# lks1248/SPH-EXA

Hardware: AMD Instinct MI355X
Metric: particle-updates/sec (whole node), Sedov -n 400, 1/2/4/8 MI355X + HBM roofline % (higher is better)
Workload: dtype f32 hydro / f64 coordinates (sph::SphTypes)

## Files before the change

### include/sphexa_hip.h

```cpp
#ifndef SPHEXA_HIP_H
#define SPHEXA_HIP_H

#include <stddef.h>
#include <stdint.h>

#ifdef __cplusplus
extern "C" {
#endif

#define SX_OK 0
#define SX_ERR_TRAVERSAL 1
#define SX_ERR_NOT_CONVERGED 2
#define SX_ERR_HIP 3
#define SX_ERR_ARG 4
#define SX_ERR_NOMEM 5

typedef struct sx_box
{
    double  lim[6];
    int32_t bnd[3];
} sx_box;

typedef struct sx_params
{
// ... 10 lines not shown
    int32_t  avClean;
    float    theta;
    double   g;
    double   eps, etaAcc;
    int32_t  propagator;
} sx_params;

typedef struct sx_fields
{
    size_t    n;
    double *  x, *y, *z;
    float *   x_m1, *y_m1, *z_m1;
    float *   vx, *vy, *vz;
    float*    rho;
    double*   u;
    float *   p, *prho, *tdpdTrho, *h, *m, *c;
    float *   ax, *ay, *az;
    double*   du;
    float*    du_m1;
    float *   c11, *c12, *c13, *c22, *c23, *c33;
    float *   mue, *mui;
    double*   temp;
    float *   cv, *xm, *kx, *divv, *curlv, *alpha, *gradh;
    uint64_t* keys;
    uint32_t* nc;
    float *   dV11, *dV12, *dV13, *dV22, *dV23, *dV33;
    float*    markRamp;
    uint8_t*  rung;
} sx_fields;

typedef struct sx_tree
{
    int32_t         numLeafNodes;
    int32_t         numNodes;
    const uint64_t* prefixes;
    const int32_t*  childOffsets;
    const int32_t*  internalToLeaf;
    const int32_t*  levelRange;
    const uint64_t* leaves;
    const uint32_t* layout;
    const double*   centers;
    const double*   sizes;
    float           searchExtFactor;
} sx_tree;

typedef struct sx_groups
{
    uint32_t        firstBody, lastBody, numGroups;
    const uint32_t* groupStart;
    const uint32_t* groupEnd;
} sx_groups;

typedef struct sx_octree
{
    uint64_t* prefixes;
    int32_t*  childOffsets;
    int32_t*  parents;
    int32_t*  levelRange;
    int32_t*  internalToLeaf;
    int32_t*  leafToInternal;
} sx_octree;

typedef struct sx_nbstats
{
    uint64_t sumNeighbors;
    uint32_t maxNeighbors;
    uint32_t numFailed;
    uint64_t sumCandidates;
    uint64_t sumUnion;
    uint32_t build;
    uint32_t maxUnion;
} sx_nbstats;

typedef struct sx_ctx sx_ctx;

int         sx_create(sx_ctx** ctx, int device);
void        sx_destroy(sx_ctx* ctx);
int         sx_set_stream(sx_ctx* ctx, void* hipStream);
void*       sx_get_stream(sx_ctx* ctx);
const char* sx_last_error(sx_ctx* ctx);
int    sx_set_exact(sx_ctx* ctx, int exact);
double sx_kernel_constant(void);
int    sx_kernel_poly(const float* v, size_t n, float* w, float* dw);
int    sx_copy_tables(sx_ctx* ctx, float* wh_host, float* whd_host);
int    sx_synchronize(sx_ctx* ctx);

void* sx_device_alloc(sx_ctx* ctx, size_t bytes);
int   sx_device_free(sx_ctx* ctx, void* ptr);
int   sx_memcpy(sx_ctx* ctx, void* dst, const void* src, size_t bytes, int kind);
int   sx_memset(sx_ctx* ctx, void* dst, int value, size_t bytes);

int sx_sfc_keys(sx_ctx* ctx, const double* x, const double* y, const double* z, uint64_t* keys, size_t n,
                const sx_box* box);
int sx_sort_keys(sx_ctx* ctx, uint64_t* keys, uint32_t* order, size_t n);
int sx_gather(sx_ctx* ctx, const uint32_t* order, size_t n, const void* src, void* dst, int elemBytes);
int sx_compute_octree(sx_ctx* ctx, const uint64_t* sortedKeys, size_t n, uint32_t bucketSize, uint64_t* leaves,
                      uint32_t* counts, int32_t capacity, int32_t* numLeaves);
int sx_build_octree(sx_ctx* ctx, const uint64_t* leaves, int32_t numLeaves, const sx_octree* out);
int sx_node_centers(sx_ctx* ctx, const uint64_t* prefixes, int32_t numNodes, const sx_box* box, double* centers,
                    double* sizes);
int sx_leaf_layout(sx_ctx* ctx, const uint32_t* counts, int32_t numLeaves, uint32_t* layout);

int sx_compute_groups(sx_ctx* ctx, uint32_t first, uint32_t last, sx_groups* groups);
int sx_spatial_groups(sx_ctx* ctx, uint32_t first, uint32_t last, const double* x, const double* y, const double* z,
                      const sx_tree* tree, const sx_box* box, float tolFactor, uint32_t* groups, uint32_t cap,
                      sx_groups* out);
int sx_set_search_mode(sx_ctx* ctx, int mode);
int sx_find_neighbors(sx_ctx* ctx, const sx_fields* f, const sx_tree* tree, const sx_box* box,
                      const sx_params* p, uint32_t first, uint32_t last, int iterate_h, sx_nbstats* stats);
int sx_export_neighbors(sx_ctx* ctx, const uint32_t* nc, uint32_t first, uint32_t last, uint32_t ngmax,
                        uint32_t* neighbors);
int sx_import_neighbors(sx_ctx* ctx, uint32_t first, uint32_t last, uint32_t ngmax, const uint32_t* neighbors);

int sx_xmass(sx_ctx* ctx, const sx_groups* g, const sx_fields* f, const sx_params* p, const sx_box* box,
             const sx_tree* tree);
int sx_xmass_only(sx_ctx* ctx, const sx_groups* g, const sx_fields* f, const sx_params* p, const sx_box* box);
int sx_ve_def_gradh(sx_ctx* ctx, const sx_groups* g, const sx_fields* f, const sx_params* p, const sx_box* box);
int sx_eos(sx_ctx* ctx, uint32_t first, uint32_t last, float mui, double gamma, const double* temp, const float* m,
           const float* kx, const float* xm, const float* gradh, float* prho, float* c, float* rho, float* p);
int sx_iad_divv_curlv(sx_ctx* ctx, const sx_groups* g, const sx_fields* f, const sx_params* p, const sx_box* box);
int sx_av_switches(sx_ctx* ctx, const sx_groups* g, const sx_fields* f, const sx_params* p, const sx_box* box,
                   double minDt);
int sx_momentum_energy(sx_ctx* ctx, const sx_groups* g, float* groupDt, const sx_fields* f, const sx_params* p,
                       const sx_box* box, float* minDtCourant);
int sx_momentum_energy_avclean(sx_ctx* ctx, const sx_groups* g, float* groupDt, const sx_fields* f,
                               const sx_params* p, const sx_box* box, float* minDtCourant);
int sx_density(sx_ctx* ctx, const sx_groups* g, const sx_fields* f, const sx_params* p, const sx_box* box,
               const sx_tree* tree);
int sx_density_only(sx_ctx* ctx, const sx_groups* g, const sx_fields* f, const sx_params* p, const sx_box* box);
int sx_eos_std(sx_ctx* ctx, uint32_t first, uint32_t last, float mui, double gamma, const double* temp,
               const float* m, float* rho, float* p, float* c);
int sx_iad(sx_ctx* ctx, const sx_groups* g, const sx_fields* f, const sx_params* p, const sx_box* box);
int sx_momentum_energy_std(sx_ctx* ctx, const sx_groups* g, const sx_fields* f, const sx_params* p,
                           const sx_box* box, float* minDtCourant);

int sx_positions(sx_ctx* ctx, uint32_t first, uint32_t last, double dt, double dt_m1, const sx_fields* f,
                 double gamma, float muiConst, const sx_box* box);
int sx_update_h(sx_ctx* ctx, uint32_t first, uint32_t last, uint32_t ng0, const uint32_t* nc, float* h);
int sx_update_h_groups(sx_ctx* ctx, const sx_groups* g, uint32_t ng0, const uint32_t* nc, float* h);

int sx_mark_ramp(sx_ctx* ctx, const sx_groups* g, const sx_fields* f, const sx_params* p, const sx_box* box,
                 float* markRamp);

#define SX_MAX_RUNGS 4
int sx_positions_rungs(sx_ctx* ctx, const sx_groups* g, float dt, const float* dt_m1, const uint8_t* rung,
                       const sx_fields* f, double gamma, double constCv, const sx_box* box);
int sx_drift_positions(sx_ctx* ctx, const sx_groups* g, float dt, float dt_back, const float* dt_m1,
                       const uint8_t* rung, const sx_fields* f, double gamma, double constCv);
int sx_group_divv_timestep(sx_ctx* ctx, float Krho, const sx_groups* g, const float* divv, float* groupDt);
int sx_group_acc_timestep(sx_ctx* ctx, float etaAcc, const sx_groups* g, const float* ax, const float* ay,
                          const float* az, float* groupDt);
int sx_store_rung(sx_ctx* ctx, const sx_groups* g, uint8_t rung, uint8_t* rungs);
int sx_max_divv(sx_ctx* ctx, uint32_t first, uint32_t last, const float* divv, float* maxDivv);

int sx_conserved_quantities(sx_ctx* ctx, const sx_fields* f, uint32_t first, uint32_t last, float muiConst,
                            double gamma, double out[9]);

int sx_gravity_upsweep(sx_ctx* ctx, const sx_fields* f, const sx_tree* tree, float theta, double* centers,
                       float* multipoles);
int sx_gravity_traverse(sx_ctx* ctx, const sx_groups* g, const sx_fields* f, const sx_tree* tree, const sx_box* box,
                        const double* centers, const float* multipoles, float G, double* egrav);
int sx_gravity_traverse_pbc(sx_ctx* ctx, const sx_groups* g, const sx_fields* f, const sx_tree* tree,
                            const sx_box* box, const double* centers, const float* multipoles, float G, int numShells,
                            double* egrav);

typedef struct
// ... 116 lines not shown
```

### sph-exa_amd/csrc/sx_capi.cpp

```cpp
#include <hip/hip_runtime.h>

#include <algorithm>
#include <cmath>
#include <cstdio>
#include <cstring>
#include <string>
#include <vector>

#include "../../include/sphexa_hip.h"
#include "sx_comm.hpp"
#include "sx_gravity.hpp"
#include "sx_hydro.hpp"
#include "sx_kernel_poly.hpp"
#include "sx_observables.hpp"
#include "sx_tree.hpp"
#include "sx_timestep.hpp"
#include "sx_turb.hpp"

using namespace sx;

namespace
{

double wharmonic(double v)
{
    if (v == 0.0) return 1.0;
    const double Pv = M_PI_2 * v;
    return std::sin(Pv) / Pv;
}

double wharmonicDerivative(double v)
{
    if (v == 0.0) return 0.0;
    const double Pv    = M_PI_2 * v;
    const double sincv = std::sin(Pv) / Pv;
    return sincv * M_PI_2 * ((std::cos(Pv) / std::sin(Pv)) - 1.0 / Pv);
}

double sinc6(double x) { return std::pow(wharmonic(x), 6.0); }
double sinc6d(double x) { return 6.0 * std::pow(wharmonic(x), 6.0 - 1) * wharmonicDerivative(x); }
double kvol(double x) { return 4.0 * M_PI * x * x * sinc6(x); }

double simpsonK()
{
    const uint64_t n = 2000;
    double a = 0, b = 2.0, h = (b - a) / double(n);
    std::vector<double> odd(n / 2), even(n / 2 - 1);
    for (uint64_t i = 0; i < odd.size(); ++i)
        odd[i] = kvol(a + double(2 * (i + 1) - 1) * h);
    for (uint64_t i = 0; i < even.size(); ++i)
        even[i] = kvol(a + double(2 * (i + 1)) * h);
    std::sort(odd.begin(), odd.end());
    std::sort(even.begin(), even.end());
    double so = 0, se = 0;
    for (double v : odd)
        so += v;
    for (double v : even)
        se += v;
    return 1.0 / (h / 3.0 * (kvol(a) + kvol(b) + 4.0 * so + 2.0 * se));
}

void makeTables(std::vector<float>& wh, std::vector<float>& whd)
{
    wh.resize(kTableSize);
    whd.resize(kTableSize);
    const float dx = (float)((2.0 - 0.0) / (kTableSize - 1));
    for (size_t i = 0; i < (size_t)kTableSize; ++i)
    {
        float nv = (float)(0.0 + (float)i * dx);
        wh[i]    = (float)sinc6((double)nv);
        whd[i]   = (float)sinc6d((double)nv);
    }
}

DevBox toDev(const sx_box* b)
{
    DevBox d{};
    for (int k = 0; k < 6; ++k)
        d.lim[k] = b->lim[k];
    d.anyPbc = 0;
    for (int k = 0; k < 3; ++k)
    {
        d.l[k]   = b->lim[2 * k + 1] - b->lim[2 * k];
        d.il[k]  = 1.0 / (b->lim[2 * k + 1] - b->lim[2 * k]);
        d.pbc[k] = b->bnd[k] == 1;
        d.fbc[k] = b->bnd[k] == 2;
        d.anyPbc |= d.pbc[k];
    }
    return d;
}

double quantMargin(const DevBox& b)
{
    double l = std::max(b.l[0], std::max(b.l[1], b.l[2]));
    return 4.0 * l / double(1u << kMaxLevel);
}

}

struct sx_ctx
{
    int         device{0};
    NsPolicy    nsPolicy;
    const uint8_t* viewActive{nullptr};
    hipStream_t own{nullptr};
    hipStream_t stream{nullptr};
    bool        exact{false};
    Arena       arena;
    float2*     wh{nullptr};
    float2*     whd{nullptr};
    double      K{0};
    std::string err;

    NbLists   nb;
    uint32_t  nbFirst{0}, nbLast{0}, nbNgmax{0};
    bool      nbValid{false};
    size_t    nbFields{0};

    uint32_t* stats{nullptr};
    uint32_t* statsHost{nullptr};
    float*    minDt{nullptr};
    unsigned* maxU{nullptr};
    float*    hostScalar{nullptr};

    float*   powTab{nullptr};
    uint32_t powTabNg0{0};

    const HydroLaunch& hydro() const { return exact ? hydro_exact() : hydro_fast(); }
};

static const float* ensurePowTab(sx_ctx* c, uint32_t ng0)
{
    if (c->powTab && c->powTabNg0 == ng0) return c->powTab;
    std::vector<float> t(kPowTable);
    const float        c0 = 1023.0f;
    const float        ex = (float)(1.0 / 10.0);
    t[0]                  = INFINITY;
    for (uint32_t nc = 1; nc < kPowTable; ++nc)
    {
        volatile float base = 1.0f + c0 * ng0 / (float)nc;
        t[nc]               = powf(base, ex);
    }
    c->powTab = c->arena.get<float>("powTab", kPowTable);
    if (hipMemcpy(c->powTab, t.data(), kPowTable * 4, hipMemcpyHostToDevice) != hipSuccess) return nullptr;
    c->powTabNg0 = ng0;
    return c->powTab;
}

static int fail(sx_ctx* c, int code, const std::string& msg)
{
    if (c) c->err = msg;
    return code;
}

#define SX_HIP(ctx, call)                                                                                              \
    do {                                                                                                               \
        hipError_t e_ = (call);                                                                                        \
        if (e_ != hipSuccess) return fail(ctx, SX_ERR_HIP, std::string(#call) + ": " + hipGetErrorString(e_));         \
    } while (0)


extern "C"
{
    void*         sx_ctx_stream_internal(sx_ctx* c) { return c->stream; }
    int           sx_ctx_exact_internal(sx_ctx* c) { return c->exact ? 1 : 0; }
    const float2* sx_ctx_table_internal(sx_ctx* c, int which) { return which ? c->whd : c->wh; }
    const float*  sx_ctx_powtab_internal(sx_ctx* c, uint32_t ng0) { return ensurePowTab(c, ng0); }
    void          sx_ctx_set_error_internal(sx_ctx* c, const char* msg) { fail(c, SX_ERR_ARG, msg); }

    int sx_kernel_poly(const float* v, size_t n, float* w, float* dw)
    {
        for (size_t k = 0; k < n; ++k)
            kernelWdW(v[k], w[k], dw[k]);
        return SX_OK;
    }

    double sx_kernel_constant(void)
    {
        static double K = simpsonK();
        return K;
    }

    int sx_create(sx_ctx** out, int device)
    {
        auto* c   = new sx_ctx;
        c->device = device;
        if (hipSetDevice(device) != hipSuccess) return fail(c, SX_ERR_HIP, "hipSetDevice"), *out = c, SX_ERR_HIP;
        SX_HIP(c, hipStreamCreateWithFlags(&c->own, hipStreamNonBlocking));
        c->stream = c->own;
        c->K      = sx_kernel_constant();
        std::vector<float> wh, whd;
        makeTables(wh, whd);
        float* tmp = c->arena.get<float>("tables.raw", 2 * kTableSize);
        SX_HIP(c, hipMemcpy(tmp, wh.data(), kTableSize * 4, hipMemcpyHostToDevice));
        SX_HIP(c, hipMemcpy(tmp + kTableSize, whd.data(), kTableSize * 4, hipMemcpyHostToDevice));
        c->wh  = c->arena.get<float2>("tables.wh", kTableSize);
        c->whd = c->arena.get<float2>("tables.whd", kTableSize);
        tablePairs(tmp, c->wh, c->stream);
        tablePairs(tmp + kTableSize, c->whd, c->stream);
        c->stats      = c->arena.get<uint32_t>("stats", kStatsWords);
        c->statsHost  = c->arena.pinned<uint32_t>("statsHost", kStatsWords);
        if (c->statsHost) std::fill(c->statsHost, c->statsHost + kStatsWords, 0u);
        c->minDt      = c->arena.get<float>("minDt", 1);
        c->maxU       = c->arena.get<unsigned>("maxU", 1);
        c->hostScalar = c->arena.pinned<float>("hostScalar", 2);
        SX_HIP(c, hipStreamSynchronize(c->stream));
        *out = c;
        return SX_OK;
    }

    void sx_destroy(sx_ctx* c)
    {
        if (!c) return;
        (void)hipDeviceSynchronize();
        c->arena.release();
        if (c->own) (void)hipStreamDestroy(c->own);
        delete c;
    }

    int sx_set_stream(sx_ctx* c, void* s)
    {
        c->stream = s ? (hipStream_t)s : c->own;
        return SX_OK;
    }
    void*       sx_get_stream(sx_ctx* c) { return c->stream; }
    const char* sx_last_error(sx_ctx* c) { return c ? c->err.c_str() : "no context"; }
    int         sx_set_exact(sx_ctx* c, int e)
    {
        c->exact = e != 0;
        return SX_OK;
    }
    int sx_synchronize(sx_ctx* c)
    {
        SX_HIP(c, hipStreamSynchronize(c->stream));
        return SX_OK;
    }

    void* sx_device_alloc(sx_ctx* c, size_t bytes)
    {
        void* p = nullptr;
        if (hipMalloc(&p, std::max<size_t>(bytes, 16)) != hipSuccess)
        {
            fail(c, SX_ERR_NOMEM, "hipMalloc failed");
            return nullptr;
        }
        return p;
    }
    int sx_device_free(sx_ctx* c, void* p)
    {
        SX_HIP(c, hipFree(p));
        return SX_OK;
// ... 90 lines not shown
    {
        g->firstBody  = first;
        g->lastBody   = last;
        g->numGroups  = (last - first + kGroupSize - 1) / kGroupSize;
        g->groupStart = nullptr;
        g->groupEnd   = nullptr;
        (void)c;
        return SX_OK;
    }

    int sx_spatial_groups(sx_ctx* c, uint32_t first, uint32_t last, const double* x, const double* y,
                          const double* z, const sx_tree* tree, const sx_box* box, float tolFactor, uint32_t* groups,
                          uint32_t cap, sx_groups* out)
    {
        if (!tree || !box || !groups || !out || last < first || (last > first && (!x || !y || !z)))
            return fail(c, SX_ERR_ARG, "sx_spatial_groups: bad arguments");
        uint32_t ng = 0;
        hipError_t e = spatialGroups(c->arena, first, last, x, y, z, tree->leaves, tree->numLeafNodes, tree->layout,
                                     toDev(box), tolFactor, groups, cap, &ng, c->stream);
        if (e == hipErrorInvalidValue) return fail(c, SX_ERR_ARG, "sx_spatial_groups: group capacity too small");
        SX_HIP(c, e);
        out->firstBody  = first;
        out->lastBody   = last;
        out->numGroups  = ng;
        out->groupStart = groups;
        out->groupEnd   = groups + 1;
        return SX_OK;
    }

    int sx_set_search_mode(sx_ctx* c, int mode)
    {
        if (mode < 0 || mode > 3) return fail(c, SX_ERR_ARG, "sx_set_search_mode: mode must be 0..3");
        c->nsPolicy.mode      = mode;
        c->nsPolicy.largeRuns = 0;
        return SX_OK;
    }

    static int findNeighborsView(sx_ctx* c, const sx_fields* f, const sx_tree* tree, const sx_box* box,
                                 const sx_params* p, uint32_t first, uint32_t last, int iterate_h, sx_nbstats* stats);

    int sx_find_neighbors(sx_ctx* c, const sx_fields* f, const sx_tree* tree, const sx_box* box, const sx_params* p,
                          uint32_t first, uint32_t last, int iterate_h, sx_nbstats* stats)
    {
        c->viewActive = nullptr;
        return findNeighborsView(c, f, tree, box, p, first, last, iterate_h, stats);
    }

    static int findNeighborsView(sx_ctx* c, const sx_fields* f, const sx_tree* tree, const sx_box* box,
                                 const sx_params* p, uint32_t first, uint32_t last, int iterate_h, sx_nbstats* stats)
    {
        if (!f || !tree || !box || !p || last < first || last > f->n)
            return fail(c, SX_ERR_ARG, "sx_find_neighbors: bad arguments");
        NsArgs a{};
        a.first          = first;
        a.last           = last;
        a.numGroups      = (last - first + kGroupSize - 1) / kGroupSize;
        a.ngmax          = p->ngmax;
        a.ng0            = p->ng0;
        a.iterateH       = iterate_h;
        a.x              = f->x;
        a.y              = f->y;
        a.z              = f->z;
        a.h              = f->h;
        a.nc             = f->nc;
        a.childOffsets   = tree->childOffsets;
        a.internalToLeaf = tree->internalToLeaf;
        a.layout         = tree->layout;
        a.centers        = tree->centers;
        a.sizes          = tree->sizes;
        a.box            = toDev(box);
        a.margin         = quantMargin(a.box);
        a.extFactor      = tree->searchExtFactor;
        a.stats          = c->stats;
        a.powTab         = ensurePowTab(c, p->ng0);
        a.prefilter      = 1;
        a.hSave          = c->arena.get<float>("ns.hsave", std::max<uint32_t>(2u * ((last - first) / kCluster + 2u), last - first));
        a.policy         = &c->nsPolicy;
        a.clStats        = c->arena.get<uint4>("ns.clstats", (a.numGroups + kClusterWaves - 1) / kClusterWaves);
        a.active         = c->viewActive;
        a.work           = c->arena.get<uint32_t>("ns.work", 16);
        a.hitMasks       = c->arena.get<uint64_t>("ns.masks", searchScratchBytes() / sizeof(uint64_t));
        if (!c->nb.reserve(c->arena, first, last, p->ngmax, true) || !a.powTab || !a.clStats || !a.work || !a.hitMasks)
            return fail(c, SX_ERR_NOMEM, "neighbor list allocation failed");
        a.setLists(c->nb);
        SX_HIP(c, hipMemsetAsync(c->stats, 0, kStatsWords * 4, c->stream));
        SX_HIP(c, findNeighbors(a, c->stream));
        SX_HIP(c, hipMemcpyAsync(c->statsHost, c->stats, kStatsWords * 4, hipMemcpyDeviceToHost, c->stream));
        SX_HIP(c, hipStreamSynchronize(c->stream));
        c->nsPolicy.observe(c->statsHost, last - first);
        c->nbFirst = first;
        c->nbLast  = last;
        c->nbNgmax = p->ngmax;
        c->nbValid = true;
        if (stats)
        {
            stats->numFailed     = c->statsHost[1];
            stats->maxNeighbors  = c->statsHost[2];
            stats->sumNeighbors  = *reinterpret_cast<uint64_t*>(c->statsHost + 4);
            stats->sumCandidates = *reinterpret_cast<uint64_t*>(c->statsHost + 6);
            stats->sumUnion      = *reinterpret_cast<uint64_t*>(c->statsHost + 8);
            stats->build         = c->nsPolicy.lastBuild;
            stats->maxUnion      = c->statsHost[12];
        }
        if (c->statsHost[0] & 1u) return fail(c, SX_ERR_TRAVERSAL, "GPU traversal stack exhausted in neighbor search");
        if (iterate_h && c->statsHost[1]) return fail(c, SX_ERR_NOT_CONVERGED, "coupled nc/h-updated failed to converge");
        return SX_OK;
    }

    int sx_export_neighbors(sx_ctx* c, const uint32_t* nc, uint32_t first, uint32_t last, uint32_t ngmax,
                               uint32_t* out)
    {
        if (!c->nbValid || first != c->nbFirst || last != c->nbLast || ngmax != c->nbNgmax)
            return fail(c, SX_ERR_ARG, "sx_export_neighbors: no matching neighbor list");
        NsArgs a{};
        a.first = first, a.last = last, a.ngmax = ngmax, a.nc = const_cast<uint32_t*>(nc);
        a.setLists(c->nb);
        SX_HIP(c, exportNeighbors(a, out, c->stream));
        return SX_OK;
    }

    int sx_import_neighbors(sx_ctx* c, uint32_t first, uint32_t last, uint32_t ngmax, const uint32_t* in)
    {
        if (!c->nb.reserve(c->arena, first, last, ngmax, false))
            return fail(c, SX_ERR_NOMEM, "neighbor list allocation failed");
        SX_HIP(c, importNeighbors(c->nb.nidx, first, last, ngmax, in, c->stream));
        c->nbFirst = first;
        c->nbLast  = last;
        c->nbNgmax = ngmax;
        c->nbValid = true;
        return SX_OK;
    }
}


namespace
{

struct Records
{
    RecX* rx;
    RecV* rv;
    RecT* rt;
    RecC* rc;
};

Records records(sx_ctx* c, size_t n)
{
    return {c->arena.get<RecX>("rec.x", n), c->arena.get<RecV>("rec.v", n), c->arena.get<RecT>("rec.t", n),
            c->arena.get<RecC>("rec.c", n)};
}

int resolveView(sx_ctx* c, const sx_groups*& g, sx_groups& tmp, size_t n, bool cachedList = true)
{
    c->viewActive = nullptr;
    if (!g) return fail(c, SX_ERR_ARG, "null group view");
    if (!g->groupStart || g->numGroups == 0) return SX_OK;
    uint8_t*  act = c->arena.get<uint8_t>("view.active", n);
    uint32_t* mm  = c->arena.get<uint32_t>("view.range", 2);
    if (!act || !mm) return fail(c, SX_ERR_NOMEM, "group view scratch");
    const uint32_t init[2] = {0xffffffffu, 0u};
    SX_HIP(c, hipMemsetAsync(act, 0, n, c->stream));
    SX_HIP(c, hipMemcpyAsync(mm, init, sizeof(init), hipMemcpyHostToDevice, c->stream));
    SX_HIP(c, viewRange(GroupArgs{g->firstBody, g->lastBody, g->numGroups, g->groupStart, g->groupEnd}, act, mm,
                        c->stream));
    uint32_t r[2];
    SX_HIP(c, hipMemcpyAsync(r, mm, sizeof(r), hipMemcpyDeviceToHost, c->stream));
    SX_HIP(c, hipStreamSynchronize(c->stream));
    tmp           = *g;
    tmp.firstBody = r[0] < r[1] ? r[0] : 0u;
    tmp.lastBody  = r[0] < r[1] ? r[1] : 0u;
    if (cachedList && c->nbValid && c->nbLast <= n && tmp.firstBody < tmp.lastBody && c->nbFirst <= tmp.firstBody &&
        tmp.lastBody <= c->nbLast)
        tmp.firstBody = c->nbFirst, tmp.lastBody = c->nbLast;
    g             = &tmp;
    c->viewActive = act;
    return SX_OK;
}

int checkList(sx_ctx* c, const sx_groups* g, const sx_params* p)
{
    if (g->firstBody >= g->lastBody) return SX_OK;
    if (!c->nbValid || g->firstBody != c->nbFirst || g->lastBody != c->nbLast || p->ngmax != c->nbNgmax)
        return fail(c, SX_ERR_ARG, "no neighbor list for this range: call sx_xmass or sx_find_neighbors first");
    return SX_OK;
}

PairArgs pairArgs(sx_ctx* c, const sx_groups* g, const sx_fields* f, const sx_params* p, const sx_box* box,
                  const Records& r)
{
    PairArgs a{};
    a.first          = g->firstBody;
    a.last           = g->lastBody;
    a.numGroups      = (g->lastBody - g->firstBody + kGroupSize - 1) / kGroupSize;
    a.ngmax          = p->ngmax;
    a.localLists     = c->nb.local;
    a.nidx           = c->nb.nidx;
    a.nloc           = c->nb.nloc;
    a.uni            = c->nb.uni;
    a.ucount         = c->nb.ucount;
    a.ucap           = c->nb.ucap;
    a.nc             = f->nc;
    a.rx             = r.rx;
    a.rv             = r.rv;
    a.rt             = r.rt;
    a.rc             = r.rc;
    a.wh             = c->wh;
    a.whd            = c->whd;
    a.box            = toDev(box);
    a.K              = p->K;
    a.xm             = f->xm;
    a.kx             = f->kx;
    a.gradh          = f->gradh;
    a.c11            = f->c11;
    a.c12            = f->c12;
    a.c13            = f->c13;
    a.c22            = f->c22;
    a.c23            = f->c23;
    a.c33            = f->c33;
    a.divv           = f->divv;
    a.curlv          = f->curlv;
    a.alpha          = f->alpha;
    a.ax             = f->ax;
    a.ay             = f->ay;
    a.az             = f->az;
    a.du             = f->du;
    a.minDt          = c->minDt;
    a.blockDt        = c->arena.get<float>("pair.blockdt", std::max<size_t>(1, (size_t(g->lastBody - g->firstBody) + kCluster - 1) / kCluster));
    a.alphamin       = p->alphamin;
    a.alphamax       = p->alphamax;
    a.decay_constant = p->decay_constant;
    a.Atmin          = p->Atmin;
    a.Atmax          = p->Atmax;
    a.ramp           = p->ramp;
    a.Kcour          = (float)p->Kcour;
    a.dV11           = f->dV11;
    a.dV12           = f->dV12;
    a.dV13           = f->dV13;
    a.dV22           = f->dV22;
    a.dV23           = f->dV23;
    a.dV33           = f->dV33;
    a.avClean        = 0;
    a.active         = c->viewActive;
    return a;
}

int markRamp(sx_ctx* c, const sx_groups* g, const sx_fields* f, const sx_params* p, const sx_box* box,
             float* markRampOut)
{
    sx_groups tmpView;
    if (int e = resolveView(c, g, tmpView, f->n)) return e;
    if (!markRampOut || !f->kx || !f->xm || !f->m) return fail(c, SX_ERR_ARG, "sx_mark_ramp: bad arguments");
    if (int e = checkList(c, g, p)) return e;
    if (g->firstBody >= g->lastBody) return SX_OK;
    const size_t n = f->n;
    Records      r = records(c, n);
    if (!r.rx) return fail(c, SX_ERR_NOMEM, "record allocation failed");
    packX(n, f->x, f->y, f->z, f->h, f->m, r.rx, c->stream);
    PairArgs a = pairArgs(c, g, f, p, box, r);
    a.markRamp = markRampOut;
    c->hydro().markRamp(a, c->stream);
    SX_HIP(c, hipGetLastError());
    return SX_OK;
}

int momentumEnergy(sx_ctx* c, const sx_groups* g, float* groupDt, const sx_fields* f, const sx_params* p,
                   const sx_box* box, float* minDtCourant, bool avClean)
{
    const sx_groups* view = g;
    sx_groups        tmp;
    if (int e = resolveView(c, g, tmp, f->n)) return e;
    if (int e = checkList(c, g, p)) return e;
    if (f->tdpdTrho) return fail(c, SX_ERR_ARG, "tdpdTrho != NULL is not supported by the VE momentum kernel");
    if (avClean && !(f->dV11 && f->dV12 && f->dV13 && f->dV22 && f->dV23 && f->dV33))
        return fail(c, SX_ERR_ARG, "avClean momentum needs the velocity gradient dV11..dV33");
    Records r = records(c, f->n);
    packX(f->n, f->x, f->y, f->z, f->h, f->m, r.rx, c->stream);
    packV(f->n, f->vx, f->vy, f->vz, f->c, r.rv, c->stream);
    packT(f->n, f->xm, f->kx, f->prho, f->alpha, r.rt, c->stream);
    packC(f->n, f->c11, f->c12, f->c13, f->c22, f->c23, f->c33, nullptr, r.rc, c->stream);
    float huge = 1e10f;
    SX_HIP(c, hipMemcpyAsync(c->minDt, &huge, 4, hipMemcpyHostToDevice, c->stream));
    PairArgs a = pairArgs(c, g, f, p, box, r);
    const bool viewGroups = groupDt && view->groupStart && view->numGroups;
// ... 660 lines not shown
```

### sph-exa_amd/csrc/sx_device.hpp

```cpp
#pragma once

#include <hip/hip_runtime.h>
#include <stdint.h>

namespace sx
{

constexpr int kWave       = 64;
constexpr int kTableSize  = 20000;
constexpr int kMaxLevel   = 21;
constexpr int kGroupSize  = 64;
constexpr int kClusterWaves = 4;
constexpr int kCluster      = kGroupSize * kClusterWaves;

__host__ __device__ constexpr uint32_t nlocWords(uint32_t ngmax) { return (ngmax + 1) / 2; }
__host__ __device__ constexpr uint32_t unionCap(uint32_t ngmax) { return kCluster * ngmax; }

struct ListsB
{
    const uint8_t*  sel;
    const uint32_t* nloc;
    const uint32_t* ucount;
    uint32_t        uoff;
};
constexpr uint8_t kListsBSel = 4;
__host__ __device__ inline bool listsB(const ListsB& b, uint32_t c) { return b.sel && (b.sel[c] & kListsBSel); }

struct DevBox
{
    double lim[6];
    double l[3];
    double il[3];
    int    pbc[3];
    int    fbc[3];
    int    anyPbc;
};

struct __attribute__((aligned(16))) RecX
{
    double x, y, z;
    float  h, m;
};
struct __attribute__((aligned(16))) RecV
{
    float vx, vy, vz, c;
};
struct __attribute__((aligned(16))) RecT
{
    float xm, kx, prho, alpha;
};
struct __attribute__((aligned(16))) RecS
{
    float rho, p, pad0, pad1;
};
struct __attribute__((aligned(16))) RecC
{
    float c11, c12, c13, c22, c23, c33, divv, vol;
};

__device__ __forceinline__ float lookup(const float2* __restrict__ tab, float v)
{
    constexpr int   numIntervals = kTableSize - 1;
    constexpr float dx           = 2.0f / numIntervals;
    constexpr float invDx        = 1.0f / dx;
    int             idx          = (int)(v * invDx);
    if (idx >= numIntervals) return 0.0f;
    float2 e          = tab[idx];
    float  derivative = e.y * invDx;
    return e.x + derivative * (v - (float)idx * dx);
}

__device__ __forceinline__ void applyPBC(const DevBox& b, float r, float& xx, float& yy, float& zz)
{
    if (b.pbc[0] && xx > r) xx = (float)((double)xx - b.l[0]);
    else if (b.pbc[0] && xx < -r) xx = (float)((double)xx + b.l[0]);
    if (b.pbc[1] && yy > r) yy = (float)((double)yy - b.l[1]);
    else if (b.pbc[1] && yy < -r) yy = (float)((double)yy + b.l[1]);
    if (b.pbc[2] && zz > r) zz = (float)((double)zz - b.l[2]);
    else if (b.pbc[2] && zz < -r) zz = (float)((double)zz + b.l[2]);
}

constexpr uint32_t kPowTable = 1u << 16;

__device__ __noinline__ float updateHFactorFar(unsigned ng0, unsigned nc)
{
    const float c0   = 1023.0f;
    const float ex   = (float)(1.0 / 10.0);
    float       base = 1.0f + c0 * ng0 / (float)nc;
    return (float)pow((double)base, (double)ex);
}

__device__ __forceinline__ float updateH(unsigned ng0, unsigned nc, float h, const float* __restrict__ powTab)
{
    const float f = nc < kPowTable ? powTab[nc] : updateHFactorFar(ng0, nc);
    return h * 0.5f * f;
}

__device__ __forceinline__ float tsKCourant(float maxvsignal, float h, float c, float Kcour)
// ... 164 lines not shown
```

### sph-exa_amd/csrc/sx_hydro.hip

```cpp
#include "sx_hydro.hpp"
#include "sx_sfc.hpp"

#ifndef SX_VARIANT
#error "SX_VARIANT must be exact or fast"
#endif

namespace sx
{
namespace SX_VARIANT
{

constexpr int kBlock = 256;
#define SX_STR2(x) #x
#define SX_STR(x) SX_STR2(x)
constexpr bool kFastClusters = SX_STR(SX_VARIANT)[0] == 'f';

#define SX_PAIR_PROLOGUE                                                                                               \
    const uint32_t gw   = (xcdBlock(blockIdx.x, gridDim.x) * kBlock + threadIdx.x) >> 6;                               \
    const uint32_t lane = threadIdx.x & 63;                                                                            \
    const uint32_t i     = a.first + gw * kGroupSize + lane;                                                           \
    const bool     valid = gw < a.numGroups && i < a.last && (!a.active || a.active[i]); \
    unsigned       cnt   = 0;                                                                                          \
    if (valid)                                                                                                         \
    {                                                                                                                  \
        unsigned c1 = a.nc[i] - 1;                                                                                     \
        cnt         = c1 < a.ngmax ? c1 : a.ngmax;                                                                     \
    }                                                                                                                  \
    const bool      lB = a.localLists && gw < a.numGroups && listsB(a.lb, gw / kClusterWaves);                       \
    const uint32_t* nb = a.localLists ? (lB ? a.lb.nloc : a.nloc) + (size_t)gw * nlocWords(a.ngmax) * kWave + lane    \
                                      : a.nidx + (size_t)gw * a.ngmax * kWave + lane;                                 \
    const uint32_t* un = a.localLists ? a.uni + (size_t)(gw / kClusterWaves) * a.ucap + (lB ? a.lb.uoff : 0u)        \
                                      : nullptr;                                                                       \
    auto nbj = [&](unsigned k) -> uint32_t {                                                                           \
        if (!a.localLists) return nb[(size_t)k * kWave];                                                               \
        uint32_t w = nb[(size_t)(k >> 1) * kWave];                                                                     \
        return un[(k & 1) ? (w >> 16) : (w & 0xffffu)];                                                                \
    };

__global__ __launch_bounds__(kBlock) void xmassKernel(PairArgs a)
{
    SX_PAIR_PROLOGUE
    if (!valid) return;
    const RecX ri    = a.rx[i];
    float      hInv  = (float)(1.0 / ri.h);
    float      h3Inv = hInv * hInv * hInv;
    float      rho0i = ri.m;
    for (unsigned k = 0; k < cnt; ++k)
    {
        uint32_t   j  = nbj(k);
        const RecX rj = a.rx[j];
        float      xx = (float)(ri.x - rj.x);
        float      yy = (float)(ri.y - rj.y);
        float      zz = (float)(ri.z - rj.z);
        applyPBC(a.box, 2.0f * ri.h, xx, yy, zz);
        float dist = sqrtf(xx * xx + yy * yy + zz * zz);
        float vloc = dist * hInv;
        float w    = lookup(a.wh, vloc);
        rho0i += w * rj.m;
    }
    a.xm[i] = (float)((double)ri.m / ((double)rho0i * a.K * (double)h3Inv));
}

__global__ __launch_bounds__(kBlock) void veDefGradhKernel(PairArgs a)
{
    SX_PAIR_PROLOGUE
    if (!valid) return;
    const RecX ri       = a.rx[i];
    const float xmassi  = a.rt[i].xm;
    float      hInv     = 1.0f / ri.h;
    float      h3Inv    = hInv * hInv * hInv;
    float      kxi      = xmassi;
    float      whomegai = -3.0f * xmassi;
    float      wrho0i   = -3.0f * ri.m;
    for (unsigned k = 0; k < cnt; ++k)
    {
        uint32_t   j  = nbj(k);
        const RecX rj = a.rx[j];
        float      xmassj = a.rt[j].xm;
        float      xx = (float)(ri.x - rj.x);
        float      yy = (float)(ri.y - rj.y);
        float      zz = (float)(ri.z - rj.z);
        applyPBC(a.box, 2.0f * ri.h, xx, yy, zz);
        float dist  = sqrtf(xx * xx + yy * yy + zz * zz);
        float vloc  = dist * hInv;
        float w     = lookup(a.wh, vloc);
        float dw    = lookup(a.whd, vloc);
        float dterh = -(3.0f * w + vloc * dw);
        kxi += w * xmassj;
        whomegai += dterh * xmassj;
        wrho0i += dterh * rj.m;
    }
    const double K = a.K;
    kxi            = (float)((double)kxi * (K * (double)h3Inv));
    whomegai       = (float)((double)whomegai * (K * (double)h3Inv * (double)hInv));
    wrho0i         = (float)((double)wrho0i * (K * (double)h3Inv * (double)hInv));
    whomegai       = (float)((double)(whomegai * ri.m / xmassi) +
                       ((double)kxi - K * (double)xmassi * (double)h3Inv) * (double)wrho0i);
    float rhoi     = kxi * ri.m / xmassi;
    float dhdrho   = -ri.h / (rhoi * 3.0f);
    a.kx[i]        = kxi;
    a.gradh[i]     = 1.0f - dhdrho * whomegai;
}

__global__ __launch_bounds__(kBlock) void iadDivvCurlvKernel(PairArgs a)
{
    SX_PAIR_PROLOGUE
    if (!valid) return;
    const RecX ri    = a.rx[i];
    const RecV vi    = a.rv[i];
    const float kxi  = a.rt[i].kx;
    float      hi    = ri.h;
    float      hiInv = 1.0f / hi;
    float      t11 = 0, t12 = 0, t13 = 0, t22 = 0, t23 = 0, t33 = 0;
    for (unsigned k = 0; k < cnt; ++k)
    {
        uint32_t   j  = nbj(k);
        const RecX rj = a.rx[j];
// ... 620 lines not shown
```

### sph-exa_amd/csrc/sx_hydro.hpp

```cpp
#pragma once

#include "sx_device.hpp"

namespace sx
{

struct EosFuse
{
    const double* temp;
    double        cv;
    double        gamma;
    float *       prho, *c;
    const float * vx, *vy, *vz, *alpha;
    RecV*         rvOut;
    RecT*         rtOut;
};

struct PairArgs
{
    uint32_t first, last, numGroups, ngmax;
    int             localLists;
    const uint32_t* nidx;
    const uint32_t* nloc;
    const uint32_t* uni;
    const uint32_t* ucount;
    uint32_t        ucap;
    ListsB          lb;
    const uint32_t* nc;
    const RecX*     rx;
    const RecV*     rv;
    const RecT*     rt;
    const RecC*     rc;
    const float2*   wh;
    const float2*   whd;
    DevBox          box;
    double          K;
    float *  xm, *kx, *gradh;
    float *  c11, *c12, *c13, *c22, *c23, *c33, *divv, *curlv;
    float*   alpha;
    float *  ax, *ay, *az;
    double*  du;
    float*   minDt;
    float*   blockDt;
    float*   groupDt;
    float  alphamin, alphamax, decay_constant;
    double        dt;
    const double* dtPtr;
    float  Atmin, Atmax, ramp, Kcour;
    float *dV11, *dV12, *dV13, *dV22, *dV23, *dV33;
    int    avClean;
    const RecS* rs;
    float* markRamp;
    const uint32_t* clusterList;
    uint32_t        listCount;
    const uint8_t* active;
    float* dtOut;
    RecT* rtOut;
    RecC* rcOut;
    uint32_t unionMax;
    EosFuse eos;
};

__device__ __forceinline__ void iadInvert(float t11, float t12, float t13, float t22, float t23, float t33, float hi,
                                          double K, float (&c)[6])
{
    auto getExp    = [](float v) { return v == 0.0f ? 0 : ilogbf(v); };
    int  tauExpSum = getExp(t11) + getExp(t12) + getExp(t13) + getExp(t22) + getExp(t23) + getExp(t33);
    const float nrm = ldexpf(1.0f, -tauExpSum / 6);
    t11 *= nrm, t12 *= nrm, t13 *= nrm, t22 *= nrm, t23 *= nrm, t33 *= nrm;
    const float det    = t11 * t22 * t33 + 2.0f * t12 * t23 * t13 - t11 * t23 * t23 - t22 * t13 * t13 - t33 * t12 * t12;
    const float factor = (float)((double)(nrm * (hi * hi * hi)) / ((double)det * K));
    c[0]               = (t22 * t33 - t23 * t23) * factor;
    c[1]               = (t13 * t23 - t33 * t12) * factor;
    c[2]               = (t12 * t23 - t22 * t13) * factor;
    c[3]               = (t11 * t33 - t13 * t13) * factor;
    c[4]               = (t13 * t12 - t11 * t23) * factor;
    c[5]               = (t11 * t22 - t12 * t12) * factor;
}

__device__ __forceinline__ float avEtaCrit(unsigned cnt)
{
    return (float)cbrt((double)32.0f * 3.14159265358979323846 / 3.0 / (double)(float)(cnt + 1));
}

template<bool EXACT>
__device__ __forceinline__ float avRvCorrection(float rx, float ry, float rz, float eta_ab, float eta_crit,
                                                const float (&gi)[6], const float (&gj)[6])
{
    const float dmy1 = rx * (gi[0] * rx + gi[1] * ry + gi[2] * rz) + (ry * (gi[3] * ry + gi[4] * rz) + rz * (gi[5] * rz));
    const float dmy2 = rx * (gj[0] * rx + gj[1] * ry + gj[2] * rz) + (ry * (gj[3] * ry + gj[4] * rz) + rz * (gj[5] * rz));
    float       dmy3 = 1.0f;
    if (eta_ab < eta_crit)
    {
        const float etaDiff = 5.0f * (eta_ab - eta_crit);
        const float arg     = -etaDiff * etaDiff;
        dmy3                = EXACT ? (float)exp((double)arg) : expf(arg);
    }
    const float A_ab   = (dmy2 != 0.0f) ? dmy1 / dmy2 : 0.0f;
    const float A_abp1 = 1.0f + A_ab;
    float       q      = 4.0f * A_ab / (A_abp1 * A_abp1);
    q                  = q < 1.0f ? q : 1.0f;
    q                  = 0.0f < q ? q : 0.0f;
    const float phi_ab = 0.5f * dmy3 * q;
    return -phi_ab * (dmy1 + dmy2);
}

struct EosArgs
{
    uint32_t      first, last;
    float         mui;
// ... 64 lines not shown
```

### sph-exa_amd/csrc/sx_hydro_cluster.hip

```cpp
#include "sx_hydro.hpp"
#include "sx_kernel_poly.hpp"
#include "sx_traverse.hpp"

namespace sx
{
namespace cluster
{

constexpr int kB = kCluster;

#ifndef SX_LEAN_DEPTH
#define SX_LEAN_DEPTH 2
#endif
#ifndef SX_ME_LEAN
#define SX_ME_LEAN true
#endif

struct Clu
{
    uint32_t        c, gw, i, iSafe, U;
    bool            valid;
    unsigned        cnt;
    uint32_t        wBeg, wEnd;
    int             part;
    int             tid;
    const uint32_t* un;
    const uint32_t* nl;
    double          ox, oy, oz;
    bool            pbc;
};

struct Rec5
{
    float4 a;
    float  s;
};
struct Rec8
{
    float4 a, b;
};
struct Rec9
{
    float4 a, b;
    float  s;
};
__device__ __forceinline__ float relc(double x, double o, const DevBox& b, int k) { return (float)foldPbc(x - o, b, k); }

template<int SPLIT>
__device__ __forceinline__ Clu setup(const PairArgs& a, float* s_red)
{
    Clu            cu;
    const int      wave = threadIdx.x >> 6, lane = threadIdx.x & 63;
    const int      sub  = wave & (kClusterWaves - 1);
    cu.part             = wave / kClusterWaves;
    cu.tid              = sub * kWave + lane;
    const uint32_t blk  = xcdBlock(blockIdx.x, gridDim.x);
    cu.c                = a.clusterList ? a.clusterList[blk] : blk;
    cu.gw               = cu.c * kClusterWaves + sub;
    const uint32_t c0   = a.first + cu.c * kCluster;
    cu.i                = c0 + cu.tid;
    cu.valid            = cu.gw < a.numGroups && cu.i < a.last && (!a.active || a.active[cu.i]);
    cu.iSafe            = cu.valid ? cu.i : c0;
    cu.cnt              = 0;
    if (cu.valid)
    {
        unsigned c1 = a.nc[cu.i] - 1;
        cu.cnt      = c1 < a.ngmax ? c1 : a.ngmax;
    }
    const uint32_t nw = (cu.cnt + 1) >> 1;
    cu.wBeg           = nw * cu.part / SPLIT;
    cu.wEnd           = nw * (cu.part + 1) / SPLIT;
    const bool lB     = listsB(a.lb, cu.c);
    cu.U              = lB ? a.lb.ucount[cu.c] : a.ucount[cu.c];
    cu.un             = a.uni + (size_t)cu.c * a.ucap + (lB ? a.lb.uoff : 0u);
    cu.nl             = (lB ? a.lb.nloc : a.nloc) + (size_t)cu.gw * nlocWords(a.ngmax) * kWave + lane;
    const RecX o      = a.rx[c0];
    cu.ox = o.x, cu.oy = o.y, cu.oz = o.z;

    const RecX r    = a.rx[cu.iSafe];
    const float h2  = 2.0f * r.h;
    float       ext = 0.0f;
    if (a.box.pbc[0]) ext = fmaxf(ext, (fabsf(relc(r.x, cu.ox, a.box, 0)) + h2) * (float)a.box.il[0]);
    if (a.box.pbc[1]) ext = fmaxf(ext, (fabsf(relc(r.y, cu.oy, a.box, 1)) + h2) * (float)a.box.il[1]);
    if (a.box.pbc[2]) ext = fmaxf(ext, (fabsf(relc(r.z, cu.oz, a.box, 2)) + h2) * (float)a.box.il[2]);
    ext = waveMax(ext);
    if (lane == 0) s_red[wave] = ext;
    __syncthreads();
    float e = s_red[0];
    for (int w = 1; w < kClusterWaves * SPLIT; ++w)
        e = fmaxf(e, s_red[w]);
    cu.pbc = __builtin_amdgcn_readfirstlane(e >= 0.49f ? 1 : 0);
    return cu;
}

template<int SPLIT, int NV>
__device__ __forceinline__ void combineShares(const Clu& cu, float (&v)[NV], float* scratch, unsigned maxMask = 0,
                                              bool scratchAliasesRecords = false)
{
    if constexpr (SPLIT > 1)
    {
        constexpr int T = SPLIT * kCluster;
        if (scratchAliasesRecords) __syncthreads();
#pragma unroll
        for (int f = 0; f < NV; ++f)
            scratch[f * T + cu.part * kCluster + cu.tid] = v[f];
        __syncthreads();
#pragma unroll
        for (int f = 0; f < NV; ++f)
        {
            float acc = scratch[f * T + cu.tid];
            for (int q = 1; q < SPLIT; ++q)
            {
                const float x = scratch[f * T + q * kCluster + cu.tid];
                acc           = ((maxMask >> f) & 1u) ? fmaxf(acc, x) : acc + x;
            }
            v[f] = acc;
        }
    }
}

template<int CH, int SPLIT, bool PF = true, bool LEAN = false, class Stage, class Load, class Compute>
__device__ __forceinline__ void neighborLoop(const Clu& cu, Stage&& stage, Load&& load, Compute&& compute,
                                             bool& resident)
{
    constexpr int NT = kB * SPLIT;
    constexpr int S  = (CH + NT - 1) / NT;
    auto          fill = [&](uint32_t b0, uint32_t b1) {
        uint32_t js[S];
#pragma unroll
        for (int s = 0; s < S; ++s)
        {
            const uint32_t u = b0 + threadIdx.x + s * NT;
            js[s]            = u < b1 ? cu.un[u] : 0u;
        }
#pragma unroll
        for (int s = 0; s < S; ++s)
        {
            const uint32_t u = b0 + threadIdx.x + s * NT;
            if (u < b1) stage(js[s], u - b0);
        }
    };

    if (cu.U <= (uint32_t)CH)
    {
        if (!resident)
        {
            fill(0, cu.U);
            __syncthreads();
            resident = true;
        }
        const uint32_t wBeg = cu.wBeg, wEnd = cu.wEnd;
        if (wBeg >= wEnd) return;
        const uint32_t* nl = cu.nl;
        if constexpr (LEAN)
        {
            const uint32_t wLast = wEnd - 1;
            auto           ld    = [&](uint32_t w) { return nl[(size_t)min(w, wLast) * kWave]; };
            constexpr int  D = SX_LEAN_DEPTH;
            uint32_t       q[D];
#pragma unroll
            for (int d = 0; d < D; ++d)
                q[d] = ld(wBeg + 1 + d);
            uint32_t       wd = nl[(size_t)wBeg * kWave];
            auto           ra = load(wd & 0xffffu);
            for (uint32_t w = wBeg;;)
            {
                const auto rb = load(wd >> 16);
                compute(ra);
                const bool odd = 2 * w + 1 < cu.cnt;
                wd             = q[0];
#pragma unroll
                for (int d = 0; d + 1 < D; ++d)
                    q[d] = q[d + 1];
                q[D - 1] = ld(w + 1 + D);
                ra             = load(wd & 0xffffu);
                if (odd) compute(rb);
                if (++w >= wEnd) break;
            }
            return;
        }
        const uint32_t  wLast = wEnd - 1;
        auto            ld    = [&](uint32_t w) {
            if constexpr (PF) return nl[(size_t)min(w, wLast) * kWave];
            else return w < wEnd ? nl[(size_t)w * kWave] : 0u;
        };
        uint32_t        q0 = ld(wBeg + 1), q1 = ld(wBeg + 2), q2 = ld(wBeg + 3);
        const uint32_t  w0 = nl[(size_t)wBeg * kWave];
        auto            a0 = load(w0 & 0xffffu);
        auto            b0 = load(w0 >> 16);
        decltype(a0)    a1, b1;
        uint32_t        w = wBeg;
        while (true)
        {
            if (PF || w + 1 < wEnd)
            {
                a1 = load(q0 & 0xffffu);
                b1 = load(q0 >> 16);
                q0 = ld(w + 4);
            }
            compute(a0);
            if (2 * w + 1 < cu.cnt) compute(b0);
            if (++w >= wEnd) break;
            if (PF || w + 1 < wEnd)
            {
                a0 = load(q1 & 0xffffu);
                b0 = load(q1 >> 16);
                q1 = ld(w + 4);
            }
            compute(a1);
            if (2 * w + 1 < cu.cnt) compute(b1);
            if (++w >= wEnd) break;
            const uint32_t t = q0;
            q0 = q2, q2 = q1, q1 = t;
        }
    }
    else
    {
        resident         = false;
        uint32_t       k    = 2 * cu.wBeg;
        const uint32_t kEnd = min(cu.cnt, 2 * cu.wEnd);
        for (uint32_t b0 = 0; b0 < cu.U; b0 += CH)
        {
            const uint32_t b1 = min(cu.U, b0 + (uint32_t)CH);
            __syncthreads();
            fill(b0, b1);
            __syncthreads();
            while (k < kEnd)
            {
                const uint32_t w = cu.nl[(size_t)(k >> 1) * kWave];
                const uint32_t p = (k & 1) ? (w >> 16) : (w & 0xffffu);
                if (p >= b1) break;
                compute(load(p - b0));
                ++k;
            }
        }
    }
}

__device__ __forceinline__ void pbcRule(const Clu& cu, const DevBox& b, float r, float& x, float& y, float& z)
{
    if (cu.pbc) applyPBC(b, r, x, y, z);
}

__device__ __forceinline__ float norm3(float a, float b, float c)
{
    const float m = fmaxf(fabsf(a), fmaxf(fabsf(b), fabsf(c)));
    if (m == 0.0f) return 0.0f;
    const float r = 1.0f / m, x = a * r, y = b * r, z = c * r;
    return m * sqrtf(x * x + (y * y + z * z));
}


template<int CH, int SPLIT>
__global__ __launch_bounds__(kB * SPLIT) void xmassKernel(PairArgs a)
{
    __shared__ float4 sP[CH];
    __shared__ float  s_red[kClusterWaves * SPLIT];
    const Clu  cu = setup<SPLIT>(a, s_red);
    const RecX ri = a.rx[cu.iSafe];
    const float xi = relc(ri.x, cu.ox, a.box, 0), yi = relc(ri.y, cu.oy, a.box, 1), zi = relc(ri.z, cu.oz, a.box, 2);
    const float hInv = 1.0f / ri.h, hInv2 = hInv * hInv, h2 = 2.0f * ri.h;
    float       rho0 = cu.part == 0 ? ri.m : 0.0f;
    bool        res  = false;
    neighborLoop<CH, SPLIT>(
        cu,
        [&](uint32_t j, uint32_t slot) {
            const RecX r = a.rx[j];
            sP[slot] = make_float4(relc(r.x, cu.ox, a.box, 0), relc(r.y, cu.oy, a.box, 1), relc(r.z, cu.oz, a.box, 2), r.m);
        },
        [&](uint32_t p) { return sP[p]; },
        [&](const float4& q) {
            float rx = xi - q.x, ry = yi - q.y, rz = zi - q.z;
            pbcRule(cu, a.box, h2, rx, ry, rz);
            rho0 += kernelWt((rx * rx + ry * ry + rz * rz) * hInv2) * q.w;
        },
        res);
    float v[1] = {rho0};
    combineShares<SPLIT>(cu, v, reinterpret_cast<float*>(sP), 0u, true);
    if (cu.valid && cu.part == 0)
    {
        const float h3Inv = hInv * hInv * hInv;
        const float xm    = (float)((double)ri.m / ((double)v[0] * a.K * (double)h3Inv));
        a.xm[cu.i]        = xm;
        if (a.rtOut) a.rtOut[cu.i] = RecT{xm, 0.0f, 0.0f, 0.0f};
    }
}

template<int CH, int SPLIT>
__global__ __launch_bounds__(kB * SPLIT) void veDefGradhKernel(PairArgs a)
{
    __shared__ float4 sP[CH];
    __shared__ float  sX[CH];
    __shared__ float  s_red[kClusterWaves * SPLIT];
    const Clu   cu     = setup<SPLIT>(a, s_red);
    const RecX  ri     = a.rx[cu.iSafe];
    const float xmassi = a.xm[cu.iSafe];
    const float xi = relc(ri.x, cu.ox, a.box, 0), yi = relc(ri.y, cu.oy, a.box, 1), zi = relc(ri.z, cu.oz, a.box, 2);
    const float hInv = 1.0f / ri.h, hInv2 = hInv * hInv, h2 = 2.0f * ri.h;
    const bool  own = cu.part == 0;
    float       kxi = own ? xmassi : 0.0f, whomegai = own ? -3.0f * xmassi : 0.0f, wrho0i = own ? -3.0f * ri.m : 0.0f;
    bool        res = false;
    neighborLoop<CH, SPLIT>(
        cu,
        [&](uint32_t j, uint32_t slot) {
            const RecX r = a.rx[j];
            sP[slot] = make_float4(relc(r.x, cu.ox, a.box, 0), relc(r.y, cu.oy, a.box, 1), relc(r.z, cu.oz, a.box, 2), r.m);
            sX[slot] = a.xm[j];
        },
        [&](uint32_t p) { return Rec5{sP[p], sX[p]}; },
        [&](const Rec5& r) {
            const float4& q      = r.a;
            const float   xmassj = r.s;
            float         rx = xi - q.x, ry = yi - q.y, rz = zi - q.z;
// ... 354 lines not shown
{
    if (Atwood < Atmin) { a_mom = xmi * xmi, b_mom = xmj * xmj; }
    else if (Atwood > Atmax) { a_mom = xmi * xmj, b_mom = a_mom; }
    else
    {
        const float sigma = ramp * (Atwood - Atmin);
        const float lxj   = __log2f(xmj);
        const float dl    = lxj - lxi;
        a_mom             = exp2f(fmaf(sigma, dl, 2.0f * lxi));
        b_mom             = exp2f(fmaf(-sigma, dl, 2.0f * lxj));
    }
}

template<bool AVC>
struct RecM
{
    float4 p, v, t, a, b, g;
    float2 g2;
};

struct MeC
{
    float4 a;
    float2 b;
};
__device__ __forceinline__ MeC meLoadC(const RecC* rc, uint32_t j)
{
    const float* p = reinterpret_cast<const float*>(rc + j);
    return MeC{*reinterpret_cast<const float4*>(p), *reinterpret_cast<const float2*>(p + 4)};
}
template<int CH, int SPLIT, bool AVC>
struct MePre
{
    static constexpr int NT = kB * SPLIT, S = (CH + NT - 1) / NT;
    static constexpr int SP = S < 2 ? S : 2;
    uint32_t c, U;
    bool     lB;
    uint32_t nc;
    uint8_t  act;
    RecX     o;
    RecX     ri;
    RecV     vi;
    RecT     ti;
    MeC      ci;
    float    gi[AVC ? 6 : 1];
    uint32_t js[S];
};
template<bool AVC>
struct MeRaw
{
    RecX  x;
    RecV  v;
    RecT  t;
    MeC   c;
    float g[AVC ? 6 : 1];
};
template<bool AVC>
__device__ __forceinline__ MeRaw<AVC> meLoadRaw(const PairArgs& a, uint32_t j)
{
    MeRaw<AVC> r;
    r.x = a.rx[j], r.v = a.rv[j], r.t = a.rt[j], r.c = meLoadC(a.rc, j);
    if constexpr (AVC)
    {
        r.g[0] = a.dV11[j], r.g[1] = a.dV12[j], r.g[2] = a.dV13[j];
        r.g[3] = a.dV22[j], r.g[4] = a.dV23[j], r.g[5] = a.dV33[j];
    }
    return r;
}

template<int CH, int SPLIT, bool AVC>
__global__ __launch_bounds__(kB * SPLIT) void momentumEnergyKernel(PairArgs a, uint32_t numClusters)
{
    __shared__ float4 sP[CH];
    __shared__ float4 sV[CH];
    __shared__ float4 sT[CH];
    __shared__ float4 sA[CH];
    __shared__ float4 sB[CH];
    __shared__ float4 sG[AVC ? CH : 1];
    __shared__ float2 sG2[AVC ? CH : 1];
    __shared__ float  s_ext[kClusterWaves * SPLIT];
    __shared__ float  s_red[kClusterWaves * SPLIT];
    using Pre                  = MePre<CH, SPLIT, AVC>;
    constexpr int  NT          = Pre::NT, S = Pre::S, SP = Pre::SP;
    const int      wave        = threadIdx.x >> 6, lane = threadIdx.x & 63;
    const int      sub         = wave & (kClusterWaves - 1);
    const int      part        = wave / kClusterWaves;
    const int      tid         = sub * kWave + lane;
    const uint32_t ucapLoad    = min((uint32_t)CH, a.ucap);
    constexpr uint32_t kNone   = ~0u;

    auto clusterAt = [&](uint32_t t) -> uint32_t {
        const uint64_t b = (uint64_t)blockIdx.x + (uint64_t)t * gridDim.x;
        if (b >= numClusters) return kNone;
        const uint32_t blk = xcdBlock((uint32_t)b, numClusters);
        return a.clusterList ? a.clusterList[blk] : blk;
    };
    auto prefetch = [&](uint32_t c) {
        Pre p;
        p.c = c;
        p.U = 0, p.nc = 1, p.act = 1, p.lB = false;
#pragma unroll
        for (int s = 0; s < S; ++s)
            p.js[s] = 0u;
        if (c == kNone) return p;
        const uint32_t c0 = __builtin_amdgcn_readfirstlane(a.first + c * kCluster), i = c0 + tid;
        const bool     in = c * kClusterWaves + sub < a.numGroups && i < a.last;
        const uint32_t iL = in ? i : c0;
        p.lB              = listsB(a.lb, c);
        p.U               = p.lB ? a.lb.ucount[c] : a.ucount[c];
        p.o               = a.rx[c0];
        p.nc              = in ? a.nc[i] : 1u;
        p.act             = (in && a.active) ? a.active[i] : (uint8_t)1;
        p.ri = a.rx[iL], p.vi = a.rv[iL], p.ti = a.rt[iL], p.ci = meLoadC(a.rc, iL);
        if constexpr (AVC)
        {
            p.gi[0] = a.dV11[iL], p.gi[1] = a.dV12[iL], p.gi[2] = a.dV13[iL];
            p.gi[3] = a.dV22[iL], p.gi[4] = a.dV23[iL], p.gi[5] = a.dV33[iL];
        }
        const uint32_t* un = a.uni + (size_t)c * a.ucap + (p.lB ? a.lb.uoff : 0u);
#pragma unroll
        for (int s = 0; s < S; ++s)
        {
            const uint32_t u = threadIdx.x + s * NT;
            p.js[s]          = u < ucapLoad ? un[u] : 0u;
        }
        return p;
    };
    auto loadRecords = [&](const Pre& p, MeRaw<AVC> (&rr)[SP]) {
        const bool use = p.c != kNone && p.U <= (uint32_t)CH;
#pragma unroll
        for (int s = 0; s < SP; ++s)
        {
            const bool ok = use && threadIdx.x + s * NT < p.U;
            rr[s]         = meLoadRaw<AVC>(a, ok ? p.js[s] : 0u);
        }
    };

    float      waveMinDt = INFINITY;
    uint32_t   t         = 0;
    Pre        cur       = prefetch(clusterAt(0));
    MeRaw<AVC> rr[SP];
    loadRecords(cur, rr);
    while (cur.c != kNone)
    {
        Clu cu;
        cu.part            = part;
        cu.tid             = tid;
        cu.c               = cur.c;
        cu.gw              = cu.c * kClusterWaves + sub;
        const uint32_t c0  = a.first + cu.c * kCluster;
        cu.i               = c0 + tid;
        cu.valid           = cu.gw < a.numGroups && cu.i < a.last && cur.act != 0;
        cu.iSafe           = cu.valid ? cu.i : c0;
        cu.cnt             = 0;
        if (cu.valid)
        {
            const unsigned c1 = cur.nc - 1;
            cu.cnt            = c1 < a.ngmax ? c1 : a.ngmax;
        }
        const uint32_t nw = (cu.cnt + 1) >> 1;
        cu.wBeg           = nw * cu.part / SPLIT;
        cu.wEnd           = nw * (cu.part + 1) / SPLIT;
        cu.U              = cur.U;
        cu.un             = a.uni + (size_t)cu.c * a.ucap + (cur.lB ? a.lb.uoff : 0u);
        cu.nl             = (cur.lB ? a.lb.nloc : a.nloc) + (size_t)cu.gw * nlocWords(a.ngmax) * kWave + lane;
        const RecX o      = cur.o;
        cu.ox = o.x, cu.oy = o.y, cu.oz = o.z;
        const RecX  ri  = cu.valid ? cur.ri : o;
        const RecV  vi  = cur.vi;
        const RecT  ti  = cur.ti;
        RecC ci6;
        ci6.c11 = cur.ci.a.x, ci6.c12 = cur.ci.a.y, ci6.c13 = cur.ci.a.z, ci6.c22 = cur.ci.a.w;
        ci6.c23 = cur.ci.b.x, ci6.c33 = cur.ci.b.y;
        {
            const float h2  = 2.0f * ri.h;
            float       ext = 0.0f;
            if (a.box.pbc[0]) ext = fmaxf(ext, (fabsf(relc(ri.x, cu.ox, a.box, 0)) + h2) * (float)a.box.il[0]);
            if (a.box.pbc[1]) ext = fmaxf(ext, (fabsf(relc(ri.y, cu.oy, a.box, 1)) + h2) * (float)a.box.il[1]);
            if (a.box.pbc[2]) ext = fmaxf(ext, (fabsf(relc(ri.z, cu.oz, a.box, 2)) + h2) * (float)a.box.il[2]);
            ext = waveMax(ext);
            if (lane == 0) s_ext[wave] = ext;
            __syncthreads();
            float e = s_ext[0];
            for (int w = 1; w < kClusterWaves * SPLIT; ++w)
                e = fmaxf(e, s_ext[w]);
            cu.pbc = __builtin_amdgcn_readfirstlane(e >= 0.49f ? 1 : 0);
        }

        auto stageRaw = [&](const MeRaw<AVC>& q, uint32_t slot) {
            const RecX& r   = q.x;
            const RecT& tq  = q.t;
            const MeC&  c6  = q.c;
            const float rho = tq.kx * r.m / tq.xm;
            sP[slot]        = make_float4(relc(r.x, cu.ox, a.box, 0), relc(r.y, cu.oy, a.box, 1),
                                   relc(r.z, cu.oz, a.box, 2), 1.0f / r.h);
            sV[slot]        = make_float4(q.v.vx, q.v.vy, q.v.vz, q.v.c);
            sT[slot]        = make_float4(r.m, tq.xm, rho, r.m * tq.prho);
            sA[slot]        = make_float4(tq.alpha, c6.a.x, c6.a.y, c6.a.z);
            sB[slot]        = make_float4(c6.a.w, c6.b.x, c6.b.y, r.m / rho);
            if constexpr (AVC)
            {
                sG[slot]  = make_float4(q.g[0], q.g[1], q.g[2], q.g[3]);
                sG2[slot] = make_float2(q.g[4], q.g[5]);
            }
        };
        bool res = false;
        if (cu.U <= (uint32_t)CH)
        {
#pragma unroll
            for (int s = 0; s < S; ++s)
            {
                const uint32_t u = threadIdx.x + s * NT;
                if (u < cu.U) stageRaw(s < SP ? rr[s < SP ? s : 0] : meLoadRaw<AVC>(a, cur.js[s]), u);
            }
            __syncthreads();
            res = true;
        }
        const Pre nxt = prefetch(clusterAt(++t));

        const float xi = relc(ri.x, cu.ox, a.box, 0), yi = relc(ri.y, cu.oy, a.box, 1), zi = relc(ri.z, cu.oz, a.box, 2);
        const float hi = ri.h, mi = ri.m, ci = vi.c, h2 = 2.0f * hi;
        const float alpha_i = ti.alpha, xmassi = ti.xm, prhoi = ti.prho;
        const float rhoi    = ti.kx * mi / xmassi;
        const float rhoiInv = 1.0f / rhoi;
        const float lxi     = __log2f(xmassi);
        const float xmi2    = xmassi * xmassi;
        const float hiInv   = 1.0f / hi;
        const float hiInv2  = hiInv * hiInv;
        const float hiInv3  = hiInv2 * hiInv;
        const float Atmin = a.Atmin, Atmax = a.Atmax, ramp = a.ramp, AtminLo = a.Atmin * (1.0f - 0x1p-20f);
        float maxvsignali = 0.0f;
        float mx = 0, my = 0, mz = 0, energy = 0, a_visc_energy = 0;
        float gradV_i[6] = {0, 0, 0, 0, 0, 0};
        float eta_crit   = 0.0f;
        if constexpr (AVC)
        {
#pragma unroll
            for (int k = 0; k < 6; ++k)
                gradV_i[k] = cur.gi[k];
            eta_crit = avEtaCrit(cu.cnt);
        }
        auto loadRec = [&](uint32_t p) {
                RecM<AVC> r;
                r.p = sP[p], r.v = sV[p], r.t = sT[p], r.a = sA[p], r.b = sB[p];
                if constexpr (AVC) r.g = sG[p], r.g2 = sG2[p];
                return r;
            };
        auto computeOne = [&](const RecM<AVC>& r) {
// ... 316 lines not shown
```

### sph-exa_amd/csrc/sx_neighbors.hip

```cpp
#include "sx_skin.hpp"
#include "sx_traverse.hpp"
#include "sx_tree.hpp"

#ifdef SX_NS_SMALL
namespace sx
{
namespace small
{
#else
namespace sx
{
#endif

#ifndef SX_NS_CCAP
#define SX_NS_CCAP 2048
#endif
constexpr int kCCap = SX_NS_CCAP;

#ifndef SX_NS_CAND_LOG2
#define SX_NS_CAND_LOG2 16
#endif
constexpr int kCandSpace = 1 << SX_NS_CAND_LOG2;
constexpr int kMaxRegions = 128;
constexpr int kCandWords = kCandSpace / 32;
// ... 782 lines not shown
            sum += __popc(mine(w));
        uint32_t incl = sum;
#pragma unroll
        for (int o = 1; o < kWave; o <<= 1)
        {
            uint32_t t = __shfl_up(incl, o, kWave);
            if (lane >= o) incl += t;
        }
        if (lane == kWave - 1) s_wsum[wave] = incl;
        __syncthreads();
        uint32_t off = 0;
        for (int w = 0; w < wave; ++w)
            off += s_wsum[w];
        for (int w = 0; w < kClusterWaves; ++w)
            ucnt += s_wsum[w];
        uint32_t run = off + incl - sum;
        for (uint32_t w = wb; w < we; ++w)
        {
            if (w * 32 >= b0) s_pre[w] = run;
            run += __popc(mine(w));
        }
        uint32_t* uni = a.uni + (size_t)c * a.ucap + a.uoff;
        run           = off + incl - sum;
        int cc = 0;
        {
            int lo = 0, hi = numCand;
            while (lo < hi)
            {
                const int mid = (lo + hi + 1) >> 1;
                if (s_cOff[mid] <= b0) lo = mid;
                else hi = mid - 1;
            }
            cc = lo;
        }
        for (uint32_t w = wb; w < we; ++w)
        {
            uint32_t bits = mine(w);
            while (bits)
            {
                const uint32_t idx = w * 32 + __builtin_ctz(bits);
                bits &= bits - 1u;
                while (s_cOff[cc + 1] <= idx)
                    ++cc;
                if (run < a.ucap - a.uoff) uni[run] = s_p0[cc] + (idx - s_cOff[cc]);
                else if (!(a.skin1 > 0.0f)) atomicOr(&a.stats[0], 1u | 8u);
                ++run;
            }
        }
        __syncthreads();
        for (int q = 0; q < nq; ++q)
        {
            const uint32_t ci = wl.tab[q][lane] & (kCandSpace - 1);
            wl.tab[q][lane]   = (uint16_t)bitRank(s_bits, s_pre, ci);
        }
        if (__ballot(nEarly > 0))
        {
            __builtin_amdgcn_s_waitcnt(0);
            const uint32_t nwl = nEarly >> 1;
            constexpr int  kRB = 8;
            for (uint32_t k0 = 0; k0 < nwl; k0 += kRB)
            {
                uint32_t v[kRB];
#pragma unroll
                for (int u = 0; u < kRB; ++u)
                    v[u] = (k0 + u < nwl) ? ll[(size_t)(k0 + u) * kWave] : 0u;
#pragma unroll
                for (int u = 0; u < kRB; ++u)
                {
                    const uint32_t k = k0 + u;
                    if (k < nwl)
                    {
                        const uint32_t lo = bitRank(s_bits, s_pre, v[u] & 0xffffu);
                        const uint32_t hp = bitRank(s_bits, s_pre, v[u] >> 16);
                        ll[(size_t)k * kWave] = lo | (hp << 16);
                    }
                }
            }
            if (nEarly & 1u) pend = bitRank(s_bits, s_pre, pend);
        }
        if (threadIdx.x == 0) a.ucount[c] = ucnt;
        __syncthreads();
        expandFinal();
        if (stored & 1u) ll[(size_t)(stored >> 1) * kWave] = pend;
    }

    if (valid && !abandoned)
    {
        a.nc[i] = count + 1;
        if (a.iterateH) a.h[i] = hi;
        if (a.rxOut) a.rxOut[i] = RecX{xi, yi, zi, hi, a.m[i]};
    }
    const unsigned           failed = (valid && a.iterateH && iteration >= 10) ? 1u : 0u;
    const unsigned           nfail  = waveSum(failed);
    const unsigned           maxCnt = waveMax(valid ? count : 0u);
    const unsigned long long nstore = waveSum((unsigned long long)(valid ? stored : 0u));
    const unsigned long long tested = waveSum(valid ? candTested : 0ull);
    if (lane == 0)
    {
        if (nfail && !abandoned) atomicAdd(&a.stats[1], nfail);
        s_cst[wave] = make_uint4(maxCnt, (uint32_t)nstore, (uint32_t)tested, 0u);
    }
    if (threadIdx.x == 0) s_next = grabCluster(a.work, numClusters, ticket);
    __syncthreads();
    if (threadIdx.x == 0 && !abandoned)
    {
        uint4 t = s_cst[0];
        for (int w = 1; w < kClusterWaves; ++w)
        {
            const uint4 u = s_cst[w];
            t.x = max(t.x, u.x), t.y += u.y, t.z += u.z;
        }
        t.w          = local ? ucnt : 0u;
        a.clStats[c] = t;
    }
    __syncthreads();
    ci = __builtin_amdgcn_readfirstlane(s_next);
    }
}


__global__ void exportKernel(NsArgs a, uint32_t* out)
{
    uint32_t i = a.first + blockIdx.x * blockDim.x + threadIdx.x;
    if (i >= a.last) return;
    uint32_t ni = i - a.first, g = ni / kGroupSize, lane = ni % kGroupSize, c = ni / kCluster;
    uint32_t cnt = a.nc[i] - 1;
    cnt          = cnt < a.ngmax ? cnt : a.ngmax;
    const uint32_t W = nlocWords(a.ngmax);
    for (uint32_t k = 0; k < a.ngmax; ++k)
    {
        uint32_t j = 0;
        if (k < cnt)
        {
            if (a.localLists)
            {
                const bool lB = listsB(a.lb, c);
                uint32_t   w  = (lB ? a.lb.nloc : a.nloc)[((size_t)g * W + k / 2) * kWave + lane];
                j = a.uni[(size_t)c * a.ucap + (lB ? a.lb.uoff : 0u) + ((k & 1) ? (w >> 16) : (w & 0xffffu))];
            }
            else { j = a.nidx[((size_t)g * a.ngmax + k) * kWave + lane]; }
        }
        out[(size_t)ni * a.ngmax + k] = j;
    }
}

__global__ void importKernel(uint32_t* nidx, uint32_t first, uint32_t last, uint32_t ngmax, const uint32_t* in)
{
    uint32_t i = first + blockIdx.x * blockDim.x + threadIdx.x;
    if (i >= last) return;
    uint32_t ni = i - first, g = ni / kGroupSize, lane = ni % kGroupSize;
    for (uint32_t k = 0; k < ngmax; ++k)
        nidx[((size_t)g * ngmax + k) * kWave + lane] = in[(size_t)ni * ngmax + k];
}

unsigned searchGrid()
{
    static unsigned grid = 0;
    if (!grid)
    {
        int dev = 0, cus = 256, perCu = 1;
        (void)hipGetDevice(&dev);
        (void)hipDeviceGetAttribute(&cus, hipDeviceAttributeMultiprocessorCount, dev);
        (void)hipOccupancyMaxActiveBlocksPerMultiprocessor(&perCu, findNeighborsKernel, kCluster, 0);
        grid = (unsigned)std::max(1, cus) * (unsigned)std::max(1, perCu);
        if (getenv("SX_NS_DEBUG_GRID")) fprintf(stderr, "search grid %u (%d per CU)\n", grid, perCu);
    }
    return grid;
}

size_t searchScratchWords() { return (size_t)searchGrid() * kClusterWaves * kBatch * kWave; }

hipError_t findNeighborsOnce(const NsArgs& a, hipStream_t s)
{
    if (a.numGroups == 0) return hipSuccess;
    const unsigned clusters = (a.numGroups + kClusterWaves - 1) / kClusterWaves;
    unsigned       grid     = std::min(searchGrid(), clusters);
    if (a.maxGrid) grid = std::min(grid, a.maxGrid);
    findNeighborsKernel<<<grid, kCluster, 0, s>>>(a);
    return hipGetLastError();
}

#ifndef SX_NS_SMALL
namespace small
{
hipError_t findNeighborsOnce(const NsArgs& a, hipStream_t s);
size_t     searchScratchWords();
}

size_t searchScratchBytes() { return std::max(searchScratchWords(), small::searchScratchWords()) * sizeof(uint64_t); }

static hipError_t reduceClusterStats(const NsArgs& a, hipStream_t s)
{
    return reduceClusterStats(a.clStats, (a.numGroups + kClusterWaves - 1) / kClusterWaves, a.stats, s);
}

hipError_t findNeighbors(const NsArgs& a, hipStream_t s)
{
    if (a.numGroups == 0) return hipSuccess;
    hipError_t e;
    if ((e = hipMemsetAsync(a.work, 0, 16 * sizeof(uint32_t), s))) return e;
    const int mode = a.policy ? a.policy->mode : 1;
    const uint32_t ncl = (a.numGroups + kClusterWaves - 1) / kClusterWaves;
    if (!a.hSave || mode == 1 || (mode == 0 && a.policy->useLarge()))
    {
        NsArgs    l    = a;
        uint32_t* over = a.hSave ? reinterpret_cast<uint32_t*>(a.hSave) : nullptr;
        l.redoList     = a.subset;
        l.redo         = over;
        if (over && (e = hipMemsetAsync(over, 0, sizeof(uint32_t), s))) return e;
        if ((e = findNeighborsOnce(l, s))) return e;
        if (over)
        {
            NsArgs t    = a;
            t.redoList  = over;
            t.coherence = 10.0f;
            t.work      = a.work + 8;
            if ((e = findNeighborsOnce(t, s))) return e;
        }
        return reduceClusterStats(a, s);
    }
    uint32_t*      redo  = reinterpret_cast<uint32_t*>(a.hSave);
// ... 43 lines not shown
```

### sph-exa_amd/csrc/sx_sim.cpp

```cpp
#include <hip/hip_runtime.h>

#include <cstdio>
#include <hipcub/hipcub.hpp>

#include <algorithm>
#include <cmath>
#include <cstring>
#include <string>
#include <type_traits>
#include <vector>

#include "../../include/sphexa_hip.h"
#include "sx_comm.hpp"
#include "sx_gravity.hpp"
#include "sx_hydro.hpp"
#include "sx_observables.hpp"
#include "sx_sim.hpp"
#include "sx_skin.hpp"
#include "sx_traverse.hpp"
#include "sx_tree.hpp"
#include "sx_turb.hpp"

using namespace sx;
using namespace sx::sim;

extern "C" void*          sx_ctx_stream_internal(sx_ctx* c);
extern "C" int            sx_ctx_exact_internal(sx_ctx* c);
extern "C" const float2*  sx_ctx_table_internal(sx_ctx* c, int which);
extern "C" const float*   sx_ctx_powtab_internal(sx_ctx* c, uint32_t ng0);
extern "C" sx::Transport* sx_comm_transport_internal(sx_comm* c);
extern "C" void           sx_ctx_set_error_internal(sx_ctx* c, const char* msg);

namespace
{

constexpr int      kHistBits   = 18;
constexpr uint32_t kChunk      = 2048;

DevBox toDevBox(const sx_box* b)
{
    DevBox d{};
    for (int k = 0; k < 6; ++k)
        d.lim[k] = b->lim[k];
    for (int k = 0; k < 3; ++k)
    {
        d.l[k]   = b->lim[2 * k + 1] - b->lim[2 * k];
        d.il[k]  = 1.0 / (b->lim[2 * k + 1] - b->lim[2 * k]);
        d.pbc[k] = b->bnd[k] == 1;
        d.fbc[k] = b->bnd[k] == 2;
        d.anyPbc |= d.pbc[k];
    }
    return d;
}

__global__ void maxAccSqKernel(const float* ax, const float* ay, const float* az, size_t first, size_t last,
                               unsigned long long* out)
{
    double v = 0.0;
    for (size_t i = first + blockIdx.x * (size_t)blockDim.x + threadIdx.x; i < last; i += (size_t)gridDim.x * blockDim.x)
    {
        double x = ax[i], y = ay[i], z = az[i], q = x * x + (y * y + z * z);
        v        = q > v ? q : v;
    }
    __shared__ double s[4];
    v = waveMax(v);
    if ((threadIdx.x & 63) == 0) s[threadIdx.x >> 6] = v;
    __syncthreads();
    if (threadIdx.x == 0)
    {
        double m = s[0];
        for (int w = 1; w < (int)(blockDim.x >> 6); ++w)
            m = s[w] > m ? s[w] : m;
        atomicMax(out, (unsigned long long)__double_as_longlong(m));
    }
}

struct __attribute__((aligned(16))) PRec
{
    double   x, y, z, temp;
    float    h, m, vx, vy, vz, xm1, ym1, zm1, dum1, alpha;
    uint64_t id;
};
static_assert(sizeof(PRec) == 80, "PRec layout");

struct __attribute__((aligned(16))) ReqBox
{
    double c[3], s[3];
    double hmax;
    int32_t owner, pad;
};


__global__ void dtCandidateKernel(Scalars* s, double Krho, double maxDtIncrease, double g, double eps, double etaAcc,
                                  int useRho)
{
    unsigned u = s->maxDivvU;
    u          = (u & 0x80000000u) ? (u & 0x7fffffffu) : ~u;
    float maxDivv   = __uint_as_float(u);
    s->minDtRho     = useRho ? Krho / (double)fabsf(maxDivv) : INFINITY;
    s->minDtCourant = (double)s->courant;
    double minDtAcc = INFINITY;
    if (g != 0.0) minDtAcc = etaAcc * sqrt(eps / sqrt(__longlong_as_double((long long)s->maxAccSqBits)));
    double m       = INFINITY;
    double cand[4] = {minDtAcc, s->minDtCourant, s->minDtRho, maxDtIncrease * s->minDt};
    for (int k = 0; k < 4; ++k)
        m = cand[k] < m ? cand[k] : m;
    s->dtCand = m;
}

__global__ void dtApplyKernel(Scalars* s)
// ... 433 lines not shown
    s->kx    = a.get<float>("kx", cap);
    s->gradh = a.get<float>("gradh", cap);
    s->prho  = a.get<float>("prho", cap);
    s->c     = a.get<float>("c", cap);
    s->divv  = a.get<float>("divv", cap);
    s->curlv = a.get<float>("curlv", cap);
    s->c11   = a.get<float>("c11", cap);
    s->c12   = a.get<float>("c12", cap);
    s->c13   = a.get<float>("c13", cap);
    s->c22   = a.get<float>("c22", cap);
    s->c23   = a.get<float>("c23", cap);
    s->c33   = a.get<float>("c33", cap);
    s->ax    = a.get<float>("ax", cap);
    s->ay    = a.get<float>("ay", cap);
    s->az    = a.get<float>("az", cap);
    s->du    = a.get<double>("du", cap);
    if (s->p.avClean)
    {
        s->dV[0] = a.get<float>("dV11", cap);
        s->dV[1] = a.get<float>("dV12", cap);
        s->dV[2] = a.get<float>("dV13", cap);
        s->dV[3] = a.get<float>("dV22", cap);
        s->dV[4] = a.get<float>("dV23", cap);
        s->dV[5] = a.get<float>("dV33", cap);
    }
    if (s->p.propagator == 1)
    {
        s->rho  = a.get<float>("rho", cap);
        s->pres = a.get<float>("p", cap);
    }
    s->rx    = a.get<RecX>("rx", cap);
    s->rv    = a.get<RecV>("rv", cap);
    s->rt    = a.get<RecT>("rt", cap);
    s->rs    = reinterpret_cast<RecS*>(s->rt);
    s->rc    = a.get<RecC>("rc", cap);
    auto spare = [&](auto*& field, const char* tag) {
        using T = std::remove_reference_t<decltype(*field)>;
        s->spares.push_back(
            {reinterpret_cast<void**>(&field), a.get<T>(std::string(tag) + ".alt", cap), (int)sizeof(T)});
    };
    spare(s->x, "x");
    spare(s->y, "y");
    spare(s->z, "z");
    spare(s->h, "h");
    spare(s->m, "m");
    spare(s->temp, "temp");
    spare(s->vx, "vx");
    spare(s->vy, "vy");
    spare(s->vz, "vz");
    spare(s->xm1, "x_m1");
    spare(s->ym1, "y_m1");
    spare(s->zm1, "z_m1");
    spare(s->dum1, "du_m1");
    spare(s->alpha, "alpha");
    spare(s->id, "id");
    if (s->p.propagator == 2)
    {
        s->rung = a.get<uint8_t>("rung", cap);
        spare(s->rung, "rung");
    }
    s->nb.reserve(a, 0, (uint32_t)cap, s->p.ngmax, true);
    s->stats      = a.get<uint32_t>("stats", kStatsWords);
    s->statsHost  = a.pinned<uint32_t>("statsHost", kStatsWords);
    s->clsHost    = a.pinned<uint32_t>("ovl.countHost", 2);
    if (s->statsHost) std::fill(s->statsHost, s->statsHost + kStatsWords, 0u);
    s->sc         = a.get<Scalars>("scalars", 1);
    s->scHost     = a.pinned<Scalars>("scalarsHost", 1);
}

PairArgs simPairArgs(sx_sim* s)
{
    PairArgs a{};
    a.lb             = s->skin.lb;
    a.first          = (uint32_t)s->first;
    a.last           = (uint32_t)s->last;
    a.numGroups      = (uint32_t)((s->last - s->first + kGroupSize - 1) / kGroupSize);
    a.ngmax          = s->p.ngmax;
    a.localLists     = s->nb.local;
    a.nidx           = s->nb.nidx;
    a.nloc           = s->nb.nloc;
    a.uni            = s->nb.uni;
    a.ucount         = s->nb.ucount;
    a.ucap           = s->nb.ucap;
    a.nc             = s->nc;
    a.rx             = s->rx;
    a.rv             = s->rv;
    a.rt             = s->rt;
    a.rc             = s->rc;
    a.wh             = sx_ctx_table_internal(s->ctx, 0);
    a.whd            = sx_ctx_table_internal(s->ctx, 1);
    a.box            = s->dbox;
    a.K              = s->p.K;
    a.xm             = s->xm;
    a.kx             = s->kx;
    a.gradh          = s->gradh;
    a.c11            = s->c11;
    a.c12            = s->c12;
    a.c13            = s->c13;
    a.c22            = s->c22;
    a.c23            = s->c23;
    a.c33            = s->c33;
    a.divv           = s->divv;
    a.curlv          = s->curlv;
    a.alpha          = s->alpha;
    a.ax             = s->ax;
    a.ay             = s->ay;
    a.az             = s->az;
    a.du             = s->du;
    a.minDt          = &s->sc->courant;
    a.blockDt        = s->mem.get<float>("pair.blockdt", std::max<size_t>(1, (s->last - s->first + kCluster - 1) / kCluster));
    a.alphamin       = s->p.alphamin;
    a.alphamax       = s->p.alphamax;
    a.decay_constant = s->p.decay_constant;
    a.dtPtr          = &s->sc->minDt;
    a.Atmin          = s->p.Atmin;
    a.Atmax          = s->p.Atmax;
    a.ramp           = s->p.ramp;
    a.Kcour          = (float)s->p.Kcour;
    a.dV11 = s->dV[0], a.dV12 = s->dV[1], a.dV13 = s->dV[2], a.dV22 = s->dV[3], a.dV23 = s->dV[4], a.dV33 = s->dV[5];
    a.rs   = s->rs;
    a.avClean = s->p.avClean ? 1 : 0;
    return a;
}

double quantMargin(const DevBox& b)
{
    return 4.0 * std::max(b.l[0], std::max(b.l[1], b.l[2])) / double(1u << kMaxLevel);
}

#define SIM_HIP(call)                                                                                                  \
    do {                                                                                                               \
        if ((call) != hipSuccess) return SX_ERR_HIP;                                                                   \
    } while (0)
#define SIM_COMM(call)                                                                                                 \
    do {                                                                                                               \
        if (!(call)) return SX_ERR_HIP;                                                                                \
    } while (0)

int sortLocals(sx_sim* s, size_t nl, hipStream_t st)
{
    uint32_t* cnt  = s->work.get<uint32_t>("sort.desc", 2);
    uint32_t* cntH = s->work.pinned<uint32_t>("sort.desch", 2);
    auto      read = [&]() -> int {
        SIM_HIP(hipMemcpyAsync(cntH, cnt, 8, hipMemcpyDeviceToHost, st));
        SIM_HIP(hipStreamSynchronize(st));
        return SX_OK;
    };
    const int bits = std::clamp(s->sortBits, 1, 63);
    uint32_t* top  = bits <= 32 ? s->work.get<uint32_t>("sort.top", nl) : nullptr;
    SIM_HIP(hipMemsetAsync(cnt, 0, 8, st));
    if (top) SIM_HIP(countDescentsTop(s->keys, nl, 63 - bits, top, cnt, st));
    else SIM_HIP(countDescents(s->keys, nl, cnt, st));
    if (int e = read()) return e;
    s->sortStats[0]++;
    if (cntH[0] == 0) return SX_OK;
    hipError_t he          = hipSuccess;
    bool       permuteKeys = false;
    uint32_t   moved       = 0;
    if (top)
    {
        SIM_HIP(sortTopBits(s->work, top, s->order, nl, bits, st));
        SIM_HIP(hipMemsetAsync(cnt, 0, 8, st));
        SIM_HIP(checkSorted(s->keys, s->order, nl, cnt, st));
        if (int e = read()) return e;
        permuteKeys = cntH[0] == 0;
        moved       = cntH[1];
// ... 821 lines not shown
    SkinGrid g{};
    g.n = kSkinGridN;
    for (int d = 0; d < 3; ++d)
    {
        g.lo[d]  = b.lim[2 * d];
        g.inv[d] = (double)kSkinGridN / b.l[d];
        g.pbc[d] = b.pbc[d];
    }
    return g;
}

uint32_t skinCapacity(uint32_t ngmax, float factor)
{
    const double f = std::pow(1.0 + factor, 3.0) * 1.15;
    const uint32_t c = (uint32_t)std::ceil(ngmax * f);
    return std::min<uint32_t>(256u, (c + 1u) & ~1u);
}

bool skinParticleBuffers(sx_sim* s, PosArgs& q, hipStream_t st)
{
    const size_t nc = (size_t)kSkinGridN * kSkinGridN * kSkinGridN;
    q.dispX = s->mem.get<float>("skin.dx", s->cap);
    q.dispY = s->mem.get<float>("skin.dy", s->cap);
    q.dispZ = s->mem.get<float>("skin.dz", s->cap);
    q.cells = s->mem.get<uint32_t>("skin.cells", kGridWords * nc);
    q.grid  = skinGrid(s->dbox);
    if (!q.dispX || !q.dispY || !q.dispZ || !q.cells) return false;
    return hipMemsetAsync(q.cells, 0xff, 3 * nc * sizeof(uint32_t), st) == hipSuccess &&
           hipMemsetAsync(q.cells + 3 * nc, 0, 3 * nc * sizeof(uint32_t), st) == hipSuccess;
}

constexpr int kSkinResync = 1000;

struct SkinCounts
{
    uint32_t clusters{0}, stale{0}, rebuilt{0}, exact{0};
};

int skinSearch(sx_sim* s, const NsArgs& na, bool reuse, hipStream_t st, float* xmOut, RecT* rtXm, SkinCounts& out)
{
    auto&          K   = s->skin;
    const uint32_t ncl = (na.numGroups + kClusterWaves - 1) / kClusterWaves;
    out                = SkinCounts{};
    out.clusters       = ncl;
    if (!reuse) K.built = K.cur;
    if (!ncl) return SX_OK;
    if (!reuse) K.ngmaxS = skinCapacity(s->p.ngmax, K.built);
    const size_t G    = kSkinGridN;
    float*       rel  = s->mem.get<float>("skin.rel", s->cap);
    float*       dx   = s->mem.get<float>("skin.dx", s->cap);
    float*       dy   = s->mem.get<float>("skin.dy", s->cap);
    float*       dz   = s->mem.get<float>("skin.dz", s->cap);
    uint32_t*   sloc = s->mem.get<uint32_t>("skin.sloc", na.numGroups * (size_t)nlocWords(K.ngmaxS) * kWave);
    uint32_t*   scnt = s->mem.get<uint32_t>("skin.scnt", s->cap);
    float*      hb   = s->mem.get<float>("skin.hb", s->cap);
    float*      acc  = s->mem.get<float>("skin.acc", ncl);
    uint32_t*   cells = s->mem.get<uint32_t>("skin.cells", kGridWords * G * G * G);
    uint32_t*   ucS   = s->mem.get<uint32_t>("skin.ucount", ncl);
    uint32_t*   l1    = s->mem.get<uint32_t>("skin.l1", ncl + 1);
    uint32_t*   l2    = s->mem.get<uint32_t>("skin.l2", ncl + 1);
    uint32_t*   l3    = s->mem.get<uint32_t>("skin.l3", ncl + 1);
    uint32_t*   hl    = s->mem.pinned<uint32_t>("skin.host", 4);
    uint8_t*    strk  = s->mem.get<uint8_t>("skin.streak", ncl);
    uint32_t*   hmask = s->mem.get<uint32_t>("skin.hitmask", na.numGroups * (size_t)kSkinMaskWords * kWave);
    uint8_t*    same  = s->mem.get<uint8_t>("skin.same", ncl);
    float2*     frz   = s->mem.get<float2>("skin.frz", ncl);
    const bool  twoSets = na.ucap / 4 >= (uint32_t)kSkinCap && !getenv("SX_SKIN_ONESET");
    uint32_t*   nlocB = twoSets ? s->mem.get<uint32_t>("skin.nlocB", na.numGroups * (size_t)nlocWords(na.ngmax) * kWave)
                                : nullptr;
    uint32_t*   ucB   = twoSets ? s->mem.get<uint32_t>("skin.ucountB", ncl) : nullptr;
    uint32_t*   hmB   = twoSets ? s->mem.get<uint32_t>("skin.hitmaskB", na.numGroups * (size_t)kSkinMaskWords * kWave)
                                : nullptr;
    if (!rel || !dx || !dy || !dz || !sloc || !scnt || !hb || !acc || !cells || !ucS || !l1 || !l2 || !l3 || !hl || !strk ||
        !hmask || !same || !frz || (twoSets && (!nlocB || !ucB || !hmB)))
        return SX_ERR_NOMEM;

    const SkinGrid g = skinGrid(s->dbox);
    SkinArgs fa{};
    fa.first = na.first, fa.last = na.last, fa.numGroups = na.numGroups, fa.ngmax = na.ngmax, fa.ng0 = na.ng0;
    fa.ngmaxS = K.ngmaxS, fa.iterateH = na.iterateH, fa.skin1 = 1.0f + K.built;
    fa.x = na.x, fa.y = na.y, fa.z = na.z, fa.h = na.h, fa.m = na.m, fa.nc = na.nc, fa.rxOut = na.rxOut;
    const uint32_t uoff = na.ucap / 2;
    fa.nloc = na.nloc, fa.uni = na.uni, fa.ucount = na.ucount, fa.ucap = na.ucap, fa.uoff = uoff, fa.ucountS = ucS;
    fa.sloc = sloc, fa.scnt = scnt, fa.hb = hb, fa.rel = rel, fa.acc = acc, fa.cells = cells, fa.grid = g;
    fa.dispX = dx, fa.dispY = dy, fa.dispZ = dz;
    fa.xmOut = xmOut, fa.rtXm = rtXm, fa.K = s->p.K;
    K.xmFused   = xmOut != nullptr;
    K.exactList = l2;
    fa.box = na.box, fa.powTab = na.powTab, fa.stats = na.stats, fa.clStats = na.clStats;
    fa.hitMask   = hmask;
    fa.same      = same;
    fa.nlocB = nlocB, fa.ucountB = ucB, fa.hitMaskB = hmB, fa.uoffB = na.ucap / 4;
    fa.frz       = getenv("SX_SKIN_NOFREEZE") ? nullptr : frz;
    fa.keepLists = reuse && K.listsKept && K.keptNloc == na.nloc && K.keptUni == na.uni && K.keptMask == hmask &&
                   K.keptSame == same && K.keptFrz == frz && K.keptNlocB == nlocB;
    K.listsKept  = false;

    NsArgs b   = na;
    b.skin1    = 1.0f + K.built;
    b.iterateH = 0;
    b.nloc     = sloc;
    b.ngmax    = K.ngmaxS;
    b.nc       = scnt;
    b.rxOut    = nullptr;
    b.uoff     = uoff;
    b.ucount   = ucS;

    SIM_HIP(hipMemsetAsync(l1, 0, 4, st));
    SIM_HIP(hipMemsetAsync(l2, 0, 4, st));
    if (!reuse)
    {
        SIM_HIP(hipMemsetAsync(strk, 0, ncl, st));
        SIM_HIP(findNeighbors(b, st));
        fa.fresh = 1;
    }
    else fa.fresh = 0;
    fa.list  = nullptr;
    fa.stale = l1;
    fa.streak = reuse ? strk : nullptr;
    fa.direct = reuse ? l2 : nullptr;
    SIM_HIP(skinFilter(fa, ncl, st));
    SIM_HIP(hipMemcpyAsync(hl, l1, 4, hipMemcpyDeviceToHost, st));
    SIM_HIP(hipMemcpyAsync(hl + 1, l2, 4, hipMemcpyDeviceToHost, st));
    SIM_HIP(hipStreamSynchronize(st));
    const uint32_t n1 = hl[0], nd = hl[1];
    uint32_t       n2 = nd;
    out.rebuilt = n1, out.stale = n1 + nd, out.exact = nd;
    NsArgs         x  = na;
    NsPolicy large;
    large.mode = 1;
    if (reuse) b.policy = x.policy = &large;
    if ((n1 || nd) && reuse)
    {
        double* c3 = s->mem.get<double>("skin.centers", 3 * (size_t)s->tree.numNodes);
        double* s3 = s->mem.get<double>("skin.sizes", 3 * (size_t)s->tree.numNodes);
        if (!c3 || !s3) return SX_ERR_NOMEM;
        SIM_HIP(skinRefreshBoxes(s->tree, na.x, na.y, na.z, na.box, c3, s3, st));
        b.centers = x.centers = c3;
        b.sizes = x.sizes = s3;
    }
    const bool early = n1 && nd && reuse && s->auxStream && s->evAuxIn && s->evAuxOut && !getenv("SX_SKIN_SERIAL_EXACT");
    if (early)
    {
        NsArgs xd   = x;
        xd.subset   = l2;
        xd.work     = s->mem.get<uint32_t>("skin.aux.work", 16);
        xd.hSave    = s->mem.get<float>("skin.aux.over", ncl + 1);
        xd.hitMasks = s->mem.get<uint64_t>("skin.aux.masks", searchScratchBytes() / sizeof(uint64_t));
        const char* sh = getenv("SX_SKIN_AUX_SHARE");
        if (!sh || atoi(sh) != 0)
        {
            const unsigned G = searchGrid();
            xd.maxGrid       = std::min(nd, G / 2);
            b.maxGrid        = G - xd.maxGrid;
        }
        if (!xd.work || !xd.hSave || !xd.hitMasks) return SX_ERR_NOMEM;
        SIM_HIP(hipEventRecord(s->evAuxIn, st));
        SIM_HIP(hipStreamWaitEvent(s->auxStream, s->evAuxIn, 0));
        SIM_HIP(findNeighbors(xd, s->auxStream));
        SIM_HIP(hipEventRecord(s->evAuxOut, s->auxStream));
    }
    uint32_t* lx = l2;
    if (n1)
    {
        b.subset  = l1;
        SIM_HIP(findNeighbors(b, st));
        fa.fresh  = 1;
        fa.list   = l1;
        if (early) SIM_HIP(hipMemsetAsync(l3, 0, 4, st));
        fa.stale  = early ? l3 : l2;
        fa.streak = nullptr;
        fa.direct = nullptr;
        SIM_HIP(skinFilter(fa, ncl, st));
        SIM_HIP(hipMemcpyAsync(hl + 2, fa.stale, 4, hipMemcpyDeviceToHost, st));
        SIM_HIP(hipStreamSynchronize(st));
        n2 = hl[2];
    }
    uint32_t n3 = 0;
    if (early)
    {
        n3 = n2, n2 = nd + n3, lx = l3;
        K.earlyExact += nd;
        SIM_HIP(hipStreamWaitEvent(st, s->evAuxOut, 0));
    }
// ... 151 lines not shown
    if (!ok) return SX_ERR_NOMEM;
    T.lat = latticeOf(M, h.modes.data());
    if (M)
    {
        SIM_HIP(hipMemcpy(T.phases, h.phases.data(), 6 * M * 8, hipMemcpyHostToDevice));
        SIM_HIP(hipMemcpy(T.modes, h.modes.data(), 3 * M * 8, hipMemcpyHostToDevice));
        SIM_HIP(hipMemcpy(T.amplitudes, h.amplitudes.data(), M * 8, hipMemcpyHostToDevice));
        if (T.lat.ok) SIM_HIP(hipMemcpy(T.slot, T.lat.slot.data(), M * 4, hipMemcpyHostToDevice));
    }
    return SX_OK;
}

int turbStep(sx_sim* s, hipStream_t st)
{
    using namespace sx::turb;
    SimTurb&     T = *s->turb;
    sx_turb&     h = *T.host;
    const size_t M = h.numModes;
    SIM_HIP(hipEventRecord(T.ev[0], st));
    if (M)
    {
        const int k = T.next;
        if (T.ringBusy[k]) SIM_HIP(hipEventSynchronize(T.ringEv[k]));
        drawNormals(h.gen, T.ring[k], 6 * M);
        SIM_HIP(hipMemcpyAsync(T.normals, T.ring[k], 6 * M * 8, hipMemcpyHostToDevice, st));
        SIM_HIP(hipEventRecord(T.ringEv[k], st));
        T.ringBusy[k] = true;
        T.next        = (k + 1) % SimTurb::kRing;
        NoiseArgs na{};
        na.dt       = &s->sc->minDt;
        na.variance = h.variance, na.decayTime = h.decayTime, na.solWeight = h.solWeight;
        na.solWeightNorm = h.solWeightNorm;
        na.numModes      = M;
        na.normals = T.normals, na.phases = T.phases, na.modes = T.modes, na.amplitudes = T.amplitudes;
        na.phasesReal = T.phasesReal, na.phasesImag = T.phasesImag;
        na.slot  = T.lat.ok ? T.slot : nullptr;
        na.table = T.table;
        SIM_HIP(advanceNoise(na, st));
    }
    SIM_HIP(hipEventRecord(T.ev[1], st));
    if (M && s->last > s->first)
    {
        StirArgs a{};
        a.first = (uint32_t)s->first, a.last = (uint32_t)s->last;
        a.numGroups = (a.last - a.first + 63) / 64;
        a.x = s->x, a.y = s->y, a.z = s->z, a.ax = s->ax, a.ay = s->ay, a.az = s->az;
        a.numModes = M, a.solWeightNorm = h.solWeightNorm;
        a.modes = T.modes, a.phasesReal = T.phasesReal, a.phasesImag = T.phasesImag, a.amplitudes = T.amplitudes;
        a.table = T.table, a.present = T.lat.present, a.w0 = T.lat.w0;
        const bool exact = sx_ctx_exact_internal(s->ctx) || !T.lat.ok;
        SIM_HIP(exact ? stirExact(a, st) : stirFast(a, st));
    }
    SIM_HIP(hipEventRecord(T.ev[2], st));
    if (s->p.g != 0.0)
    {
        SIM_HIP(hipMemsetAsync(&s->sc->maxAccSqBits, 0, sizeof(unsigned long long), st));
        maxAccSq(s, st);
    }
    return SX_OK;
}

}

extern "C"
{

    int sx_sim_create(sx_sim** out, sx_ctx* ctx, size_t capacity, const sx_params* p, const sx_box* box,
                      uint32_t bucketSize)
    {
        if (p->propagator < 0 || p->propagator > 2) return SX_ERR_ARG;
        if (p->g != 0.0 && (box->bnd[0] == 1 || box->bnd[1] == 1 || box->bnd[2] == 1))
        {
            const bool allPbc = box->bnd[0] == 1 && box->bnd[1] == 1 && box->bnd[2] == 1;
            const double lx = box->lim[1] - box->lim[0], ly = box->lim[3] - box->lim[2], lz = box->lim[5] - box->lim[4];
            if (!allPbc || lx != ly || lx != lz || p->propagator == 2) return SX_ERR_ARG;
        }
        auto* s   = new sx_sim;
        s->ctx    = ctx;
        s->p      = *p;
        s->box    = *box;
        s->dbox   = toDevBox(box);
        s->bucket = bucketSize;
        s->cap    = capacity;
        allocFields(s, capacity);
        if (s->p.propagator == 2) allocBdt(s);
        if (s->mem.failed())
        {
            delete s;
            return SX_ERR_NOMEM;
        }
        const char* names[] = {"sync",         "FindNeighbors", "XMass",          "VeDefGradh", "EOS",
                               "IadDivvCurlv", "AVswitches",    "MomentumEnergy", "Gravity",    "UpdateQuantities"};
        s->stageNames.assign(std::begin(names), std::end(names));
        s->ev.resize(s->stageNames.size() + 1);
        for (auto& e : s->ev)
            (void)hipEventCreate(&e);
        s->stageMs.assign(s->stageNames.size(), 0.f);
        const char* knames[] = {"findNeighbors", "xmass",          "veDefGradh", "iadDivvCurlv",
                                "avSwitches",    "momentumEnergy", "gravity"};
        s->kernelNames.assign(std::begin(knames), std::end(knames));
        s->kev.resize(2 * s->kernelNames.size());
        for (auto& e : s->kev)
            (void)hipEventCreate(&e);
        s->kernelMs.assign(s->kernelNames.size(), 0.f);
        if (hipStreamCreateWithFlags(&s->commStream, hipStreamNonBlocking) != hipSuccess) s->commStream = nullptr;
        (void)hipEventCreateWithFlags(&s->evProd, hipEventDisableTiming);
        (void)hipEventCreateWithFlags(&s->evComm, hipEventDisableTiming);
        (void)hipEventCreateWithFlags(&s->evStats, hipEventDisableTiming);
        {
            int least = 0, greatest = 0;
            (void)hipDeviceGetStreamPriorityRange(&least, &greatest);
            const char* ap = getenv("SX_SKIN_AUX_PRIO");
            const int   pr = ap && atoi(ap) == 0 ? least : greatest;
            if (hipStreamCreateWithPriority(&s->auxStream, hipStreamNonBlocking, pr) != hipSuccess) s->auxStream = nullptr;
        }
        (void)hipEventCreateWithFlags(&s->evAuxIn, hipEventDisableTiming);
        (void)hipEventCreateWithFlags(&s->evAuxOut, hipEventDisableTiming);
        Scalars init{1e-6, 1e-6, 0.0, INFINITY, INFINITY, 0.0, 1e10f, 0, 0.0, 0ull, 0u};
        (void)hipMemcpy(s->sc, &init, sizeof(Scalars), hipMemcpyHostToDevice);
        *out = s;
        return SX_OK;
    }

    void sx_sim_destroy(sx_sim* s)
    {
        if (!s) return;
        (void)hipDeviceSynchronize();
        for (auto& e : s->ev)
            (void)hipEventDestroy(e);
        for (auto& e : s->kev)
            (void)hipEventDestroy(e);
        if (s->evProd) (void)hipEventDestroy(s->evProd);
        if (s->evComm) (void)hipEventDestroy(s->evComm);
        if (s->evStats) (void)hipEventDestroy(s->evStats);
        if (s->commStream) (void)hipStreamDestroy(s->commStream);
        if (s->evAuxIn) (void)hipEventDestroy(s->evAuxIn);
        if (s->evAuxOut) (void)hipEventDestroy(s->evAuxOut);
        if (s->auxStream) (void)hipStreamDestroy(s->auxStream);
        turbDestroy(s->turb);
        delete s;
    }

    int sx_sim_set_comm(sx_sim* s, sx_comm* c)
    {
        if (s->turb)
        {
            sx_ctx_set_error_internal(s->ctx, "sx_sim_set_comm: a stirred sim (sx_sim_set_turbulence) runs on one rank");
            return SX_ERR_ARG;
        }
        sx::Transport* T = sx_comm_transport_internal(c);
        if (T && T->size() > 1)
        {
            const size_t P  = (size_t)T->size();
            const bool   ok = s->work.get<uint32_t>("dom.bins", size_t(1) << kHistBits) &&
                            s->work.get<uint64_t>("dom.split", P + 1) && s->work.get<uint64_t>("dom.seg", P + 1) &&
                            s->work.get<uint64_t>("dom.cnt", 2 * P) && s->work.pinned<uint64_t>("dom.cnth", 2 * P) &&
                            s->work.get<uint32_t>("dom.agree", 1) && s->work.pinned<uint32_t>("dom.agreeh", 1) &&
                            s->work.get<unsigned>("dom.hflag", 1) && s->work.pinned<unsigned>("dom.hflagh", 1) &&
                            s->work.pinned<uint32_t>("dom.errh", 1);
            if (!ok) return SX_ERR_NOMEM;
        }
        s->keysFresh  = false;
        s->skin.valid = false;
        s->comm       = T;
        s->commHandle = c;
        return SX_OK;
// ... 923 lines not shown
```

### sph-exa_amd/csrc/sx_skin.hip

```cpp
#include "sx_kernel_poly.hpp"
#include "sx_skin.hpp"
#include "sx_traverse.hpp"

namespace sx
{

namespace
{

constexpr int kWalkPF  = 8;
constexpr int kWalkBlocks = (nlocWords(256) + kWalkPF - 1) / kWalkPF;
constexpr int kB       = kCluster;

__device__ __forceinline__ int cellIndex(double v, const SkinGrid& g, int d) { return gridCell(v, g, d); }

__device__ __forceinline__ float keepOrZero(float v, bool k)
{
    return __builtin_bit_cast(float, __builtin_bit_cast(uint32_t, v) & (0u - (uint32_t)k));
}

__device__ __forceinline__ float norm3up(float x, float y, float z)
{
    return sqrtf(fmaf(x, x, fmaf(y, y, z * z))) * (1.0f + 0x1p-18f) + 1e-30f;
}
// ... 223 lines not shown
        if (lane == 0) s_red[wave] = gmx;
        __syncthreads();
        float g = s_red[0];
        for (int w = 1; w < kClusterWaves; ++w)
            g = fmaxf(g, s_red[w]);
        A = a.acc[c] + g;
        __syncthreads();
    }
    auto withinSkin = [&](float h) { return 2.0f * h + di + A <= Ri * (1.0f - kEps); };
    bool frozen = false;
    {
        const bool bad  = valid && (scount > a.ngmaxS || !withinSkin(hi));
        const bool thin = !a.fresh && valid && 2.0f * hi + 2.0f * (di + A) > Ri * (1.0f - kEps);
        const float e    = di + A + kEps * Ri;
        const bool  melt = valid && !(e + 2.0f * hi < fref.x && e - 2.0f * hi < fref.y);
        const uint32_t v = blockBits((bad ? 1u : 0u) | (thin ? 2u : 0u) | (melt ? 4u : 0u));
        if ((v & 1u) || U > (uint32_t)kSkinCap || U > a.ucap - a.uoff)
        {
            if (threadIdx.x == 0) pushStale(a, c);
            return;
        }
        if ((v & 2u) && threadIdx.x == 0) atomicAdd(&a.stats[13], 1u);
        frozen = mayFreeze && !(v & 4u);
    }
    int      iteration = 0;
    unsigned count = 0, stored = 0;
    const float mi   = a.m[iS];
    float    rho0    = mi;
    bool     kept    = frozen;
    uint32_t ue      = 0;
    float    frzK    = -INFINITY;
    const float xr = (float)foldPbc(xi - ox, a.box, 0), yr = (float)foldPbc(yi - oy, a.box, 1),
                zr = (float)foldPbc(zi - oz, a.box, 2);
    auto setLists = [&](uint32_t k) { return (k ? a.nlocB : a.nloc) + (size_t)gw * nlocWords(a.ngmax) * kWave + lane; };
    auto setUnion = [&](uint32_t k) { return a.uni + (size_t)c * a.ucap + (k ? a.uoffB : 0u); };
    auto setCount = [&](uint32_t k) { return k ? a.ucountB + c : a.ucount + c; };
    auto setMask  = [&](uint32_t k) {
        uint32_t* m = k ? a.hitMaskB : a.hitMask;
        return m ? m + (size_t)gw * kSkinMaskWords * kWave + lane : nullptr;
    };
    const uint32_t* const ll = setLists(lcur);
    auto stage = [&](const uint32_t* list, uint32_t n) -> float {
        constexpr int S = (kSkinCap + kB - 1) / kB;
        uint32_t      js[S];
#pragma unroll
        for (int q = 0; q < S; ++q)
        {
            js[q] = list[min(threadIdx.x + q * kB, n ? n - 1u : 0u)];
        }
        double px[S], py[S], pz[S];
        float  mq[S];
#pragma unroll
        for (int q = 0; q < S; ++q)
            px[q] = a.x[js[q]], py[q] = a.y[js[q]], pz[q] = a.z[js[q]], mq[q] = a.m[js[q]];
        float pm = 0.0f;
#pragma unroll
        for (int q = 0; q < S; ++q)
        {
            const uint32_t u = threadIdx.x + q * kB;
            if (u < n)
            {
                const float fx = (float)foldPbc(px[q] - ox, a.box, 0);
                const float fy = (float)foldPbc(py[q] - oy, a.box, 1);
                const float fz = (float)foldPbc(pz[q] - oz, a.box, 2);
                s_rec[u]       = make_float4(fx, fy, fz, mq[q]);
                pm             = fmaxf(pm, fabsf(fx) + fabsf(fy) + fabsf(fz));
            }
        }
        pm = waveMax(pm);
        if (lane == 0) s_red[wave] = pm;
        __syncthreads();
        float r = s_red[0];
        for (int w = 1; w < kClusterWaves; ++w)
            r = fmaxf(r, s_red[w]);
        return r;
    };

    if (frozen)
    {
        ue = __builtin_amdgcn_readfirstlane(*setCount(lcur));
        (void)stage(setUnion(lcur), ue);
        count  = valid ? a.nc[i] - 1u : 0u;
        stored = min(count, a.ngmax);
        if (a.xmOut && valid)
        {
            const float    hInv = 1.0f / hi, hInv2 = hInv * hInv;
            const uint32_t nw = (stored + 1) >> 1, last = nw ? nw - 1 : 0u;
            constexpr int  PF = kWalkPF;
            uint32_t       nx[PF];
#pragma unroll
            for (int u = 0; u < PF; ++u)
                nx[u] = ll[(size_t)min((uint32_t)u, last) * kWave];
            for (uint32_t w0 = 0; w0 < nw; w0 += PF)
            {
                uint32_t cw[PF];
#pragma unroll
                for (int u = 0; u < PF; ++u)
                {
                    cw[u] = nx[u];
                    nx[u] = ll[(size_t)min(w0 + PF + u, last) * kWave];
                }
#pragma unroll
                for (int u = 0; u < PF; ++u)
                {
                    const uint32_t w = w0 + u;
#pragma unroll
                    for (int h2 = 0; h2 < 2; ++h2)
                    {
                        const float4 q  = s_rec[min(h2 ? cw[u] >> 16 : cw[u] & 0xffffu, (uint32_t)kSkinCap - 1u)];
                        const float  dx = q.x - xr, dy = q.y - yr, dz = q.z - zr;
                        const float  r2 = fmaf(dx, dx, fmaf(dy, dy, dz * dz));
                        rho0 += keepOrZero(kernelWt(r2 * hInv2) * q.w, 2 * w + h2 < stored);
                    }
                }
            }
        }
    }
    else
    {

    const uint32_t* un   = a.uni + (size_t)c * a.ucap + a.uoff;
    const float     pmax = stage(un, U);

    const uint32_t  WS = nlocWords(a.ngmaxS);
    const uint32_t* sl = a.sloc + (size_t)gw * WS * kWave + lane;
    const unsigned  ngmin     = a.ng0 / 4;
    bool            active    = valid;
    auto walk = [&](auto&& begin, auto&& visit, auto&& end) {
        if (!valid) return;
        const uint32_t nw   = (scount + 1) >> 1;
        const uint32_t last = nw ? nw - 1 : 0u;
        constexpr int  PF   = kWalkPF;
        uint32_t       nx[PF];
#pragma unroll
        for (int u = 0; u < PF; ++u)
            nx[u] = sl[(size_t)min((uint32_t)u, last) * kWave];
        for (uint32_t w0 = 0, b = 0; w0 < nw; w0 += PF, ++b)
        {
            uint32_t cw[PF];
#pragma unroll
            for (int u = 0; u < PF; ++u)
            {
                cw[u] = nx[u];
                nx[u] = sl[(size_t)min(w0 + PF + u, last) * kWave];
            }
            begin(b);
#pragma unroll
            for (int u = 0; u < PF; ++u)
            {
                const uint32_t w = w0 + u;
                visit(cw[u] & 0xffffu, 2 * u, 2 * w < scount);
                visit(min(cw[u] >> 16, (uint32_t)kSkinCap - 1u), 2 * u + 1, 2 * w + 1 < scount);
            }
            end(b);
        }
    };
    float          r2f = 0, tol = 0;
    double         radSq = 0;
    bool           safe = true, usePbc = false;
    auto test = [&](uint32_t p, float4 q, bool inr, float& r2, float& t) -> bool {
        const float dx = q.x - xr, dy = q.y - yr, dz = q.z - zr;
        r2             = fmaf(dx, dx, fmaf(dy, dy, dz * dz));
        t              = r2 - r2f;
        bool        hit = t < 0.0f;
        if (inr & ((!safe) | (fabsf(t) <= tol)))
        {
            const uint32_t j  = un[p];
// ... 75 lines not shown
            if (threadIdx.x == 0) pushStale(a, c);
            return;
        }
        if (!blockAny(again)) break;
    }
    if (valid && safe && iteration == 0)
    {
        const float g = fminf(fmaxf(0.0f, tmin - tol) / ((Ri + 2.0f * hi) * (1.0f + 0x1p-20f)), Ri - 2.0f * hi);
        frzK          = (g * (1.0f - 0x1p-20f) + di + A) * (1.0f - 0x1p-22f);
    }

    const uint32_t nbl = valid ? (((scount + 1) >> 1) + kWalkPF - 1) / kWalkPF : 0u;
    auto           maskWord = [&](uint32_t k) {
        const uint32_t lo = s_bm[2 * k][threadIdx.x];
        return 2 * k + 1 < nbl ? lo | ((uint32_t)s_bm[2 * k + 1][threadIdx.x] << 16) : lo;
    };
    auto sameBits = [&](const uint32_t* hm) -> bool {
        constexpr int MW = (kWalkBlocks + 1) / 2;
        const uint32_t nmw = (nbl + 1) >> 1;
        uint32_t       prev[MW];
#pragma unroll
        for (int k = 0; k < MW; ++k)
            prev[k] = hm[(size_t)min((uint32_t)k, nmw ? nmw - 1 : 0u) * kWave];
        bool diff = false;
#pragma unroll
        for (int k = 0; k < MW; ++k)
            if ((uint32_t)k < nmw) diff |= prev[k] != maskWord(k);
        return !blockAny(diff);
    };
    uint32_t lnew = lstate;
    uint32_t ltgt = lcur;
    const bool otherValid = a.nlocB && a.hitMask && ((lstate >> (1u - lcur)) & 1u);
    if (otherValid && sameBits(setMask(1u - lcur)))
    {
        kept = true, ltgt = 1u - lcur;
        lnew = (lstate & 3u) | (ltgt ? kListsBSel : 0u);
    }
    if (!kept && a.hitMask && curValid) kept = sameBits(setMask(lcur));
    if (!kept)
    {
        ltgt = a.nlocB ? 1u - lcur : 0u;
        lnew = (curValid && ltgt != lcur ? 1u << lcur : 0u) | (1u << ltgt) | (ltgt ? kListsBSel : 0u);
    }

    ue = kept ? __builtin_amdgcn_readfirstlane(*setCount(ltgt)) : 0u;
    if (!kept)
    {
        const uint32_t B  = (U + kB - 1) / kB;
        const uint32_t b0 = min(U, threadIdx.x * B), b1 = min(U, b0 + B);
        uint32_t       sum = 0;
        for (uint32_t u = b0; u < b1; ++u)
            sum += s_hit[u];
        uint32_t incl = sum;
#pragma unroll
        for (int o = 1; o < kWave; o <<= 1)
        {
            const uint32_t t = __shfl_up(incl, o, kWave);
            if (lane >= o) incl += t;
        }
        if (lane == kWave - 1) s_wsum[wave] = incl;
        __syncthreads();
        uint32_t run = incl - sum;
        for (int w = 0; w < wave; ++w)
            run += s_wsum[w];
        for (int w = 0; w < kClusterWaves; ++w)
            ue += s_wsum[w];
        uint32_t* ux = setUnion(ltgt);
        for (uint32_t u0 = b0; u0 < b1; u0 += 8)
        {
            uint32_t jj[8];
#pragma unroll
            for (int q = 0; q < 8; ++q)
                jj[q] = un[min(u0 + q, U - 1u)];
#pragma unroll
            for (int q = 0; q < 8; ++q)
                if (u0 + q < b1)
                {
                    s_rank[u0 + q] = (uint16_t)run;
                    if (s_hit[u0 + q]) ux[run++] = jj[q];
                }
        }
        __syncthreads();
    }
    if (!kept)
    {
        uint32_t* const lw = setLists(ltgt);
        unsigned st = 0;
        uint32_t pend = 0, bits = 0;
        walk([&](uint32_t b) { bits = s_bm[b][threadIdx.x]; },
             [&](uint32_t p, int e, bool) {
                 const bool     keep = ((bits >> e) & 1u) != 0;
                 const uint32_t r    = s_rank[p];
                 const bool     odd  = (st & 1u) != 0;
                 if (keep && odd) lw[(size_t)(st >> 1) * kWave] = pend | (r << 16);
                 pend = (keep && !odd) ? r : pend;
                 st += keep ? 1u : 0u;
             },
             [](uint32_t) {});
        if (st & 1u) lw[(size_t)(st >> 1) * kWave] = pend;
        if (uint32_t* const hm = setMask(ltgt))
            for (uint32_t k = 0; 2 * k < nbl; ++k)
                hm[(size_t)k * kWave] = maskWord(k);
        if (threadIdx.x == 0) *setCount(ltgt) = ue;
    }
    if (threadIdx.x == 0 && a.same && lnew != lstate) a.same[c] = (uint8_t)lnew;
    }

    if (valid)
    {
        if (!frozen)
        {
            a.nc[i] = count + 1;
        }
        if (a.iterateH && iteration > 0) a.h[i] = hi;
        if (a.rxOut) a.rxOut[i] = RecX{xi, yi, zi, hi, a.m[i]};
        if (a.fresh) a.hb[i] = h0;
        a.rel[i] = di;
        if (a.xmOut)
        {
            const float hInv  = 1.0f / hi;
            const float h3Inv = hInv * hInv * hInv;
            const float xm    = (float)((double)mi / ((double)rho0 * a.K * (double)h3Inv));
            a.xmOut[i]        = xm;
            if (a.rtXm) a.rtXm[i] = RecT{xm, 0.0f, 0.0f, 0.0f};
        }
    }
    if (threadIdx.x == 0)
    {
        a.acc[c]    = a.fresh ? 0.0f : A;
        if (a.streak && !a.fresh) a.streak[c] = 0;
    }
    const unsigned           failed = (valid && a.iterateH && iteration >= 10) ? 1u : 0u;
    const unsigned           nfail  = waveSum(failed);
    const unsigned           maxCnt = waveMax(valid ? count : 0u);
    const unsigned long long nst    = waveSum((unsigned long long)(valid ? stored : 0u));
    const unsigned long long walked = waveSum((unsigned long long)scount);
    const float kp = waveMin(valid ? frzK + 2.0f * hi : INFINITY), km = waveMin(valid ? frzK - 2.0f * hi : INFINITY);
    if (lane == 0)
    {
        if (nfail) atomicAdd(&a.stats[1], nfail);
        s_cst[wave]  = make_uint4(maxCnt, (uint32_t)nst, (uint32_t)walked, __float_as_uint(kp));
        s_wsum[wave] = __float_as_uint(km);
    }
    __syncthreads();
    if (threadIdx.x == 0)
    {
        if (a.frz && !frozen)
        {
            float2 f = make_float2(__uint_as_float(s_cst[0].w), __uint_as_float(s_wsum[0]));
            for (int w = 1; w < kClusterWaves; ++w)
                f.x = fminf(f.x, __uint_as_float(s_cst[w].w)), f.y = fminf(f.y, __uint_as_float(s_wsum[w]));
            a.frz[c] = f;
        }
        uint4 t = s_cst[0];
        for (int w = 1; w < kClusterWaves; ++w)
            t.x = max(t.x, s_cst[w].x), t.y += s_cst[w].y, t.z += s_cst[w].z;
        t.y |= (kept ? 0x80000000u : 0u) | (frozen ? 0x40000000u : 0u);
        t.w          = ue;
        a.clStats[c] = t;
    }
}

inline unsigned grid1(size_t n, int b = 256) { return (unsigned)((n + b - 1) / b); }

}

hipError_t skinFilter(const SkinArgs& a, uint32_t numClusters, hipStream_t s)
// ... 34 lines not shown
```

### sph-exa_amd/csrc/sx_skin.hpp

```cpp
#pragma once

#include "sx_tree.hpp"

namespace sx
{

using SkinGrid = DispGrid;

constexpr int kSkinGridN = 64;
constexpr int kSkinCap   = 1920;
constexpr uint32_t kSkinMaskWords = 8;

struct SkinArgs
{
    uint32_t first, last, numGroups, ngmax, ng0;
    uint32_t ngmaxS;
    int      iterateH;
    int      fresh;
    float    skin1;
    const double *x, *y, *z;
    float*       h;
    const float* m;
    uint32_t*    nc;
    RecX*        rxOut;
    uint32_t*       nloc;
    uint32_t*       uni;
    uint32_t*       ucount;
    uint32_t        ucap;
    uint32_t        uoff;
    const uint32_t* ucountS;
    const uint32_t* sloc;
    const uint32_t* scnt;
    float*          hb;
    float*          rel;
    const float *   dispX, *dispY, *dispZ;
    float*          acc;
    const uint32_t* cells;
    SkinGrid        grid;
    const uint32_t* list;
    uint32_t*       stale;
    uint8_t*        streak;
    uint32_t*       direct;
    uint32_t*       hitMask;
    uint8_t*        same;
    int             keepLists;
    uint32_t*       nlocB;
    uint32_t*       ucountB;
    uint32_t*       hitMaskB;
    uint32_t        uoffB;
    float2*         frz;
    DevBox          box;
    const float*    powTab;
    float*          xmOut;
    RecT*           rtXm;
    double          K;
    uint32_t*       stats;
    uint4*          clStats;
};

hipError_t skinFilter(const SkinArgs& a, uint32_t numClusters, hipStream_t s);
hipError_t skinRefreshBoxes(const DevTree& t, const double* x, const double* y, const double* z, const DevBox& box,
                            double* centers, double* sizes, hipStream_t s, bool withCells = false);
hipError_t skinMarkStale(const uint32_t* list, uint32_t numClusters, float* acc, hipStream_t s);
hipError_t reduceClusterStats(const uint4* clStats, uint32_t numClusters, uint32_t* stats, hipStream_t s);

}
```

### sph-exa_amd/csrc/sx_tree.hpp

```cpp
#pragma once

#include <algorithm>
#include <map>
#include <string>
#include <vector>

#include "sx_device.hpp"

namespace sx
{

class Arena
{
public:
    ~Arena() { release(); }

    template<class T>
    T* get(const std::string& tag, size_t count)
    {
        return static_cast<T*>(getBytes(tag, std::max<size_t>(1, count) * sizeof(T), false));
    }
    template<class T>
    T* pinned(const std::string& tag, size_t count)
    {
// ... 11 lines not shown
        for (auto& kv : bufs_)
        {
            if (kv.second.host) (void)hipHostFree(kv.second.ptr);
            else (void)hipFree(kv.second.ptr);
        }
        bufs_.clear();
    }
    bool failed() const { return failed_; }

private:
    struct Buf
    {
        void*  ptr{nullptr};
        size_t bytes{0};
        bool   host{false};
    };
    void* getBytes(const std::string& tag, size_t bytes, bool host)
    {
        auto it = bufs_.find(tag);
        if (it != bufs_.end() && it->second.bytes >= bytes) return it->second.ptr;
        if (it != bufs_.end())
        {
            (void)hipDeviceSynchronize();
            if (it->second.host) (void)hipHostFree(it->second.ptr);
            else (void)hipFree(it->second.ptr);
            bufs_.erase(it);
        }
        size_t alloc = bytes + bytes / 8 + 256;
        void*  p     = nullptr;
        hipError_t e = host ? hipHostMalloc(&p, alloc) : hipMalloc(&p, alloc);
        if (e != hipSuccess)
        {
            failed_ = true;
            return nullptr;
        }
        bufs_[tag] = Buf{p, alloc, host};
        return p;
    }
    std::map<std::string, Buf> bufs_;
    bool                       failed_{false};
};

struct DevTree
{
    int       numLeaves{0}, numNodes{0}, numInternal{0};
    uint64_t* leaves{nullptr};
    uint32_t* counts{nullptr};
    uint32_t* layout{nullptr};
    uint64_t* prefixes{nullptr};
    int32_t*  childOffsets{nullptr};
    int32_t*  parents{nullptr};
    int32_t*  levelRange{nullptr};
    int32_t*  internalToLeaf{nullptr};
    int32_t*  leafToInternal{nullptr};
    double*   centers{nullptr};
    double*   sizes{nullptr};
    std::vector<int32_t> levelRangeHost;

    int  parentsSize() const { return std::max(1, (numNodes - 1) / 8); }
    void reserve(Arena& a)
    {
        leaves         = a.get<uint64_t>("dt.leaves", numLeaves + 1);
        counts         = a.get<uint32_t>("dt.counts", numLeaves + 1);
        layout         = a.get<uint32_t>("dt.layout", numLeaves + 1);
        prefixes       = a.get<uint64_t>("dt.prefixes", numNodes);
        childOffsets   = a.get<int32_t>("dt.childOffsets", numNodes + 1);
        parents        = a.get<int32_t>("dt.parents", parentsSize());
        levelRange     = a.get<int32_t>("dt.levelRange", kMaxLevel + 2);
        internalToLeaf = a.get<int32_t>("dt.internalToLeaf", numNodes);
        leafToInternal = a.get<int32_t>("dt.leafToInternal", numNodes);
        centers        = a.get<double>("dt.centers", 3 * (size_t)numNodes);
        sizes          = a.get<double>("dt.sizes", 3 * (size_t)numNodes);
    }
};

struct NbLists
{
    int       local{0};
    uint32_t  first{0}, last{0}, ngmax{0}, ucap{0};
    uint32_t* nidx{nullptr};
    uint32_t* nloc{nullptr};
    uint32_t* uni{nullptr};
    uint32_t* ucount{nullptr};

    size_t groups() const { return (size_t(last - first) + kGroupSize - 1) / kGroupSize; }
    size_t clusters() const { return (size_t(last - first) + kCluster - 1) / kCluster; }
    static bool localPossible(uint32_t ngmax) { return unionCap(ngmax) <= 65536u; }
    bool reserve(Arena& a, uint32_t f, uint32_t l, uint32_t ng, bool wantLocal)
    {
        first = f, last = l, ngmax = ng;
        local = (wantLocal && localPossible(ng)) ? 1 : 0;
        size_t gr = std::max<size_t>(1, groups()), cl = std::max<size_t>(1, clusters());
        if (local)
        {
            ucap   = unionCap(ng);
            nloc   = a.get<uint32_t>("nb.nloc", gr * nlocWords(ng) * kWave);
            uni    = a.get<uint32_t>("nb.uni", cl * ucap);
            ucount = a.get<uint32_t>("nb.ucount", cl);
            return nloc && uni && ucount;
        }
        nidx = a.get<uint32_t>("nb.nidx", gr * ng * kWave);
        return nidx != nullptr;
    }
};

constexpr int kStatsWords = 28;

struct NsPolicy
{
    int      mode{0};
    int      largeRuns{0};
    uint64_t prevStored{0};
    uint32_t prevTargets{0};
    uint32_t lastBuild{0};

    void observe(const uint32_t* statsHost, uint32_t targets)
    {
        lastBuild = statsHost[10] ? 2u : (statsHost[11] ? 0u : 1u);
        const uint64_t clusters = (targets + kCluster - 1) / kCluster;
        if (8ull * statsHost[10] > clusters) largeRuns = 64;
        prevStored  = *reinterpret_cast<const uint64_t*>(statsHost + 4);
        prevTargets = targets;
    }
    bool useLarge()
    {
        if (largeRuns > 0)
        {
            --largeRuns;
            return true;
        }
        return false;
    }
};

struct NsArgs
{
    uint32_t        first, last, numGroups, ngmax, ng0;
    int             iterateH;
    const double *  x, *y, *z;
    float*          h;
    uint32_t*       nc;
    uint32_t*       nidx;
    int             localLists;
    ListsB          lb;
    uint32_t*       nloc;
    uint32_t*       uni;
    uint32_t*       ucount;
    uint32_t        ucap;
    const int32_t*  childOffsets;
    const int32_t*  internalToLeaf;
    const uint32_t* layout;
    const double*   centers;
    const double*   sizes;
    DevBox          box;
    double          margin;
    double          extFactor;
    const float*    powTab;
    int             prefilter;
    uint32_t*       stats;
    const uint8_t*  active;
    uint4*          clStats;
    float*          hSave;
    NsPolicy*       policy;
    uint32_t*       redo;
    const uint32_t* redoList;
    int             forceOverflow;
    float           coherence;
    uint32_t*       work;
    uint64_t*       hitMasks;
    uint32_t        maxGrid;
    RecX*           rxOut;
    const float*    m;
    float           skin1;
    uint32_t        uoff;
    const uint32_t* subset;

    void setLists(const NbLists& L)
    {
        localLists = L.local;
        nidx       = L.nidx;
        nloc       = L.nloc;
        uni        = L.uni;
        ucount     = L.ucount;
        ucap       = L.ucap;
    }
};

hipError_t launchSfcKeys(const double* x, const double* y, const double* z, uint64_t* keys, size_t n,
                         const DevBox& b, hipStream_t s);
hipError_t sortKeys(Arena& arena, uint64_t* keys, uint32_t* order, size_t n, hipStream_t s);
hipError_t countDescents(const uint64_t* keys, size_t n, uint32_t* out, hipStream_t s);
uint64_t*  sortKeysBits(Arena& arena, const uint64_t* keys, uint32_t* order, size_t n, int beginBit, hipStream_t s,
                        hipError_t& e);
hipError_t countDescentsTop(const uint64_t* keys, size_t n, int shift, uint32_t* top, uint32_t* out, hipStream_t s);
hipError_t sortTopBits(Arena& arena, const uint32_t* top, uint32_t* order, size_t n, int bits, hipStream_t s);
hipError_t checkSorted(const uint64_t* keys, const uint32_t* order, size_t n, uint32_t* out, hipStream_t s);
hipError_t gather(const uint32_t* order, size_t n, const void* src, void* dst, int elemBytes, hipStream_t s);
constexpr int kMaxGatherFields = 16;
struct GatherSet
{
    int         count;
    const void* src[kMaxGatherFields];
    void*       dst[kMaxGatherFields];
    int         bytes[kMaxGatherFields];
};
hipError_t gatherMany(const uint32_t* order, size_t n, const GatherSet& set, hipStream_t s);
hipError_t movedCount(const uint32_t* order, size_t n, uint32_t* count, hipStream_t s);
hipError_t permuteMoved(const uint32_t* order, size_t n, const GatherSet& set, char* tmp, hipStream_t s);
hipError_t buildTree(Arena& arena, const uint64_t* keys, size_t n, uint32_t bucket, const DevBox& box, DevTree& t,
                     hipStream_t s);
hipError_t nodeCenters(const uint64_t* prefixes, int numNodes, const DevBox& b, double* centers, double* sizes,
                       hipStream_t s);
hipError_t leafLayout(Arena& arena, const uint32_t* counts, int numLeaves, uint32_t* layout, hipStream_t s);
hipError_t maxFloat(const float* v, uint32_t first, uint32_t last, unsigned* out, hipStream_t s);
void       packX(size_t n, const double* x, const double* y, const double* z, const float* h, const float* m, RecX* out,
                 hipStream_t s);
void       packV(size_t n, const float* vx, const float* vy, const float* vz, const float* c, RecV* out, hipStream_t s);
void       packT(size_t n, const float* xm, const float* kx, const float* prho, const float* alpha, RecT* out,
                 hipStream_t s);
void       packC(size_t n, const float* c11, const float* c12, const float* c13, const float* c22, const float* c23,
                 const float* c33, const float* divv, RecC* out, hipStream_t s, const float* xm = nullptr,
                 const float* kx = nullptr);
void       packS(size_t n, const float* rho, const float* p, RecS* out, hipStream_t s);
void       tablePairs(const float* t, float2* out, hipStream_t s);

hipError_t spatialGroups(Arena& arena, uint32_t first, uint32_t last, const double* x, const double* y,
                         const double* z, const uint64_t* leaves, int numLeaves, const uint32_t* layout,
                         const DevBox& b, float tolFactor, uint32_t* groups, uint32_t cap, uint32_t* numGroups,
                         hipStream_t s);
hipError_t findNeighbors(const NsArgs& a, hipStream_t s);
size_t     searchScratchBytes();
unsigned   searchGrid();
hipError_t exportNeighbors(const NsArgs& a, uint32_t* out, hipStream_t s);
hipError_t importNeighbors(uint32_t* nidx, uint32_t first, uint32_t last, uint32_t ngmax, const uint32_t* in,
                           hipStream_t s);

}
```

### sph-exa_amd/python/sphexa_amd/__init__.py

```python
import ctypes as C
import os
import re

import numpy as np

HERE = os.path.dirname(os.path.abspath(__file__))
PKG = os.path.dirname(os.path.dirname(HERE))
ROOT = os.path.dirname(PKG)
LIB_PATH = os.environ.get("SPHEXA_AMD_LIB") or os.path.join(PKG, "lib", "libsphexa_hip.so")
HEADER = os.path.join(ROOT, "include", "sphexa_hip.h")

SX_OK, SX_ERR_TRAVERSAL, SX_ERR_NOT_CONVERGED, SX_ERR_HIP, SX_ERR_ARG, SX_ERR_NOMEM = range(6)
KTABLE = 20000
GROUP = 64


class SxBox(C.Structure):
    _fields_ = [("lim", C.c_double * 6), ("bnd", C.c_int32 * 3)]


class SxParams(C.Structure):
    _fields_ = [("K", C.c_double), ("ng0", C.c_uint32), ("ngmax", C.c_uint32), ("Kcour", C.c_double),
                ("Krho", C.c_double), ("gamma", C.c_double), ("muiConst", C.c_float), ("alphamin", C.c_float),
                ("alphamax", C.c_float), ("decay_constant", C.c_float), ("Atmin", C.c_float),
# ... 23 lines not shown
                ("sizes", _P), ("searchExtFactor", C.c_float)]


class SxEwaldSettings(C.Structure):
    _fields_ = [("numReplicaShells", C.c_int), ("lCut", C.c_double), ("hCut", C.c_double), ("alphaScale", C.c_double),
                ("smallRScaleFactor", C.c_double)]

    def __init__(self, numReplicaShells=1, lCut=2.6, hCut=2.8, alphaScale=2.0, smallRScaleFactor=3.0e-3):
        super().__init__(numReplicaShells, lCut, hCut, alphaScale, smallRScaleFactor)


class SxGroups(C.Structure):
    _fields_ = [("firstBody", C.c_uint32), ("lastBody", C.c_uint32), ("numGroups", C.c_uint32),
                ("groupStart", _P), ("groupEnd", _P)]


class SxTimestep(C.Structure):
    _fields_ = [("nextDt", C.c_float), ("elapsedDt", C.c_float), ("totDt", C.c_float), ("numRungs", C.c_int),
                ("substep", C.c_int), ("rungRanges", C.c_uint32 * 5), ("dt_m1", C.c_float * 4),
                ("dt_drift", C.c_float * 4)]


class SxTurbSettings(C.Structure):
    _fields_ = [("solWeight", C.c_double), ("stMaxModes", C.c_uint64), ("Lbox", C.c_double),
                ("stEnergyPrefac", C.c_double), ("stMachVelocity", C.c_double), ("epsilon", C.c_double),
                ("rngSeed", C.c_uint64), ("stSpectForm", C.c_uint32), ("powerLawExp", C.c_double),
                ("anglesExp", C.c_double)]

    def __init__(self, **kw):
        super().__init__()
        lib().sx_turb_default_settings(C.byref(self))
        for k, v in kw.items():
            if k not in dict(self._fields_):
                raise TypeError(f"unknown turbulence setting {k!r}")
            setattr(self, k, v)


class SxOctree(C.Structure):
    _fields_ = [("prefixes", _P), ("childOffsets", _P), ("parents", _P), ("levelRange", _P),
                ("internalToLeaf", _P), ("leafToInternal", _P)]


class SxNbStats(C.Structure):
    _fields_ = [("sumNeighbors", C.c_uint64), ("maxNeighbors", C.c_uint32), ("numFailed", C.c_uint32),
                ("sumCandidates", C.c_uint64), ("sumUnion", C.c_uint64), ("build", C.c_uint32),
                ("maxUnion", C.c_uint32)]


DTYPES = {k: np.float32 for k, _ in FIELD_ORDER}
DTYPES.update(x=np.float64, y=np.float64, z=np.float64, u=np.float64, du=np.float64, temp=np.float64,
              keys=np.uint64, nc=np.uint32, rung=np.uint8)

_lib = None

ALLTOALLV_CB = C.CFUNCTYPE(C.c_int, C.c_void_p, C.c_void_p, C.POINTER(C.c_uint64), C.c_void_p,
                           C.POINTER(C.c_uint64))
ALLREDUCE_CB = C.CFUNCTYPE(C.c_int, C.c_void_p, C.c_void_p, C.c_uint64, C.c_int)


def header_symbols():
    txt = open(HEADER).read()
    txt = re.sub(r"/\*.*?\*/", "", txt, flags=re.S)
    return sorted(set(re.findall(r"\b(sx_[a-z0-9_]+)\s*\(", txt)))


def lib():
    global _lib
    if _lib is not None:
        return _lib
    if not os.path.exists(LIB_PATH):
        raise FileNotFoundError(f"{LIB_PATH} not built (run __graft_entry__.build() or make -C sph-exa_amd)")
    L = C.CDLL(LIB_PATH)
    vp, i32, u32, sz = C.c_void_p, C.c_int32, C.c_uint32, C.c_size_t
    sig = {
        "sx_create": (C.c_int, [C.POINTER(vp), C.c_int]),
        "sx_destroy": (None, [vp]),
        "sx_set_stream": (C.c_int, [vp, vp]),
        "sx_get_stream": (vp, [vp]),
        "sx_last_error": (C.c_char_p, [vp]),
        "sx_set_exact": (C.c_int, [vp, C.c_int]),
        "sx_kernel_constant": (C.c_double, []),
        "sx_copy_tables": (C.c_int, [vp, vp, vp]),
        "sx_kernel_poly": (C.c_int, [vp, C.c_size_t, vp, vp]),
        "sx_synchronize": (C.c_int, [vp]),
        "sx_device_alloc": (vp, [vp, sz]),
        "sx_device_free": (C.c_int, [vp, vp]),
        "sx_memcpy": (C.c_int, [vp, vp, vp, sz, C.c_int]),
        "sx_memset": (C.c_int, [vp, vp, C.c_int, sz]),
        "sx_sfc_keys": (C.c_int, [vp, vp, vp, vp, vp, sz, C.POINTER(SxBox)]),
        "sx_sort_keys": (C.c_int, [vp, vp, vp, sz]),
        "sx_gather": (C.c_int, [vp, vp, sz, vp, vp, C.c_int]),
        "sx_compute_octree": (C.c_int, [vp, vp, sz, u32, vp, vp, i32, C.POINTER(i32)]),
        "sx_build_octree": (C.c_int, [vp, vp, i32, C.POINTER(SxOctree)]),
        "sx_node_centers": (C.c_int, [vp, vp, i32, C.POINTER(SxBox), vp, vp]),
        "sx_leaf_layout": (C.c_int, [vp, vp, i32, vp]),
        "sx_compute_groups": (C.c_int, [vp, u32, u32, C.POINTER(SxGroups)]),
        "sx_set_search_mode": (C.c_int, [vp, C.c_int]),
        "sx_mark_ramp": (C.c_int, [vp, C.POINTER(SxGroups), C.POINTER(SxFields), C.POINTER(SxParams),
                                   C.POINTER(SxBox), vp]),
        "sx_positions_rungs": (C.c_int, [vp, C.POINTER(SxGroups), C.c_float, vp, vp, C.POINTER(SxFields), C.c_double,
                                         C.c_double, C.POINTER(SxBox)]),
        "sx_drift_positions": (C.c_int, [vp, C.POINTER(SxGroups), C.c_float, C.c_float, vp, vp, C.POINTER(SxFields),
                                         C.c_double, C.c_double]),
        "sx_group_divv_timestep": (C.c_int, [vp, C.c_float, C.POINTER(SxGroups), vp, vp]),
        "sx_group_acc_timestep": (C.c_int, [vp, C.c_float, C.POINTER(SxGroups), vp, vp, vp, vp]),
        "sx_store_rung": (C.c_int, [vp, C.POINTER(SxGroups), C.c_uint8, vp]),
        "sx_rung_timestep": (C.c_int, [vp, vp, vp, u32, C.c_float, vp, C.POINTER(SxTimestep)]),
        "sx_minimum_group_dt": (C.c_int, [vp, C.POINTER(SxTimestep), vp, vp, u32, vp, C.POINTER(C.c_float), vp]),
        "sx_extract_groups": (C.c_int, [vp, C.POINTER(SxGroups), vp, u32, u32, vp, vp]),
        "sx_spatial_groups": (C.c_int, [vp, u32, u32, vp, vp, vp, C.POINTER(SxTree), C.POINTER(SxBox), C.c_float,
                                        vp, u32, C.POINTER(SxGroups)]),
        "sx_find_neighbors": (C.c_int, [vp, C.POINTER(SxFields), C.POINTER(SxTree), C.POINTER(SxBox),
                                        C.POINTER(SxParams), u32, u32, C.c_int, C.POINTER(SxNbStats)]),
        "sx_export_neighbors": (C.c_int, [vp, vp, u32, u32, u32, vp]),
        "sx_import_neighbors": (C.c_int, [vp, u32, u32, u32, vp]),
        "sx_xmass": (C.c_int, [vp, C.POINTER(SxGroups), C.POINTER(SxFields), C.POINTER(SxParams), C.POINTER(SxBox),
                               C.POINTER(SxTree)]),
        "sx_xmass_only": (C.c_int, [vp, C.POINTER(SxGroups), C.POINTER(SxFields), C.POINTER(SxParams),
                                    C.POINTER(SxBox)]),
        "sx_ve_def_gradh": (C.c_int, [vp, C.POINTER(SxGroups), C.POINTER(SxFields), C.POINTER(SxParams),
                                      C.POINTER(SxBox)]),
        "sx_eos": (C.c_int, [vp, u32, u32, C.c_float, C.c_double, vp, vp, vp, vp, vp, vp, vp, vp, vp]),
        "sx_iad_divv_curlv": (C.c_int, [vp, C.POINTER(SxGroups), C.POINTER(SxFields), C.POINTER(SxParams),
                                        C.POINTER(SxBox)]),
        "sx_av_switches": (C.c_int, [vp, C.POINTER(SxGroups), C.POINTER(SxFields), C.POINTER(SxParams),
                                     C.POINTER(SxBox), C.c_double]),
        "sx_momentum_energy": (C.c_int, [vp, C.POINTER(SxGroups), vp, C.POINTER(SxFields), C.POINTER(SxParams),
                                         C.POINTER(SxBox), C.POINTER(C.c_float)]),
        "sx_momentum_energy_avclean": (C.c_int, [vp, C.POINTER(SxGroups), vp, C.POINTER(SxFields),
                                                 C.POINTER(SxParams), C.POINTER(SxBox), C.POINTER(C.c_float)]),
        "sx_density": (C.c_int, [vp, C.POINTER(SxGroups), C.POINTER(SxFields), C.POINTER(SxParams),
                                 C.POINTER(SxBox), C.POINTER(SxTree)]),
        "sx_density_only": (C.c_int, [vp, C.POINTER(SxGroups), C.POINTER(SxFields), C.POINTER(SxParams),
                                      C.POINTER(SxBox)]),
        "sx_eos_std": (C.c_int, [vp, u32, u32, C.c_float, C.c_double, vp, vp, vp, vp, vp]),
        "sx_iad": (C.c_int, [vp, C.POINTER(SxGroups), C.POINTER(SxFields), C.POINTER(SxParams), C.POINTER(SxBox)]),
        "sx_momentum_energy_std": (C.c_int, [vp, C.POINTER(SxGroups), C.POINTER(SxFields), C.POINTER(SxParams),
                                             C.POINTER(SxBox), C.POINTER(C.c_float)]),
        "sx_positions": (C.c_int, [vp, u32, u32, C.c_double, C.c_double, C.POINTER(SxFields), C.c_double,
                                   C.c_float, C.POINTER(SxBox)]),
        "sx_update_h": (C.c_int, [vp, u32, u32, u32, vp, vp]),
        "sx_update_h_groups": (C.c_int, [vp, vp, u32, vp, vp]),
        "sx_max_divv": (C.c_int, [vp, u32, u32, vp, C.POINTER(C.c_float)]),
        "sx_sim_create": (C.c_int, [C.POINTER(vp), vp, sz, C.POINTER(SxParams), C.POINTER(SxBox), u32]),
        "sx_sim_destroy": (None, [vp]),
        "sx_sim_init_sedov": (C.c_int, [vp, u32]),
        "sx_sim_set_state": (C.c_int, [vp, sz] + [vp] * 15 + [C.c_double, C.c_double]),
        "sx_sim_fields": (C.c_int, [vp, C.POINTER(SxFields), C.POINTER(vp)]),
        "sx_sim_size": (sz, [vp]),
        "sx_sim_step": (C.c_int, [vp]),
        "sx_sim_scalars": (C.c_int, [vp, C.POINTER(C.c_double)]),
        "sx_sim_stage_times": (C.c_int, [vp, C.POINTER(C.c_float), C.c_int, C.POINTER(C.c_char_p)]),
        "sx_sim_last_stats": (C.c_int, [vp, C.POINTER(SxNbStats)]),
        "sx_sim_kernel_times": (C.c_int, [vp, C.POINTER(C.c_float), C.c_int, C.POINTER(C.c_char_p)]),
        "sx_sim_set_comm": (C.c_int, [vp, vp]),
        "sx_sim_gravity_stats": (C.c_int, [vp, C.POINTER(C.c_uint64)]),
        "sx_sim_gravity_interactions": (C.c_int, [vp, C.POINTER(C.c_uint64)]),
        "sx_sim_set_gravity_counting": (C.c_int, [vp, C.c_int]),
        "sx_sim_conserved": (C.c_int, [vp, C.POINTER(C.c_double)]),
        "sx_conserved_quantities": (C.c_int, [vp, C.POINTER(SxFields), u32, u32, C.c_float, C.c_double,
                                              C.POINTER(C.c_double)]),
        "sx_sim_init_sedov_rank": (C.c_int, [vp, u32, C.c_int, C.c_int]),
        "sx_sim_layout": (C.c_int, [vp, C.POINTER(C.c_uint64)]),
        "sx_sim_set_overlap": (C.c_int, [vp, C.c_int]),
        "sx_sim_overlap_stats": (C.c_int, [vp, C.POINTER(C.c_uint32)]),
        "sx_sim_timestep": (C.c_int, [vp, C.POINTER(SxTimestep)]),
# ... 153 lines not shown
        modes, amp, ph = np.empty(3 * m), np.empty(m), np.empty(6 * m)
        self.L.sx_turb_get_arrays(self.h, modes.ctypes.data, amp.ctypes.data, ph.ctypes.data)
        return dict(modes=modes, amplitudes=amp, phases=ph)

    def rng_state(self):
        n = self.L.sx_turb_get_rng(self.h, None, 0)
        buf = C.create_string_buffer(n + 1)
        self.L.sx_turb_get_rng(self.h, buf, n + 1)
        return buf.value.decode()

    def state(self):
        sc, ar = self.scalars(), self.arrays()
        d = {"turbulence::" + k: np.float64(v) for k, v in sc.items()}
        d["turbulence::numModes"] = np.uint64(self.num_modes)
        d.update({"turbulence::" + k: v for k, v in ar.items()})
        d["rngEngineState"] = np.frombuffer(self.rng_state().encode(), dtype=np.uint8).copy()
        return {k: d[k] for k in TURBULENCE_ATTRIBUTES}

    @staticmethod
    def _state_args(state):
        sc = (C.c_double * 4)(*[float(np.asarray(state["turbulence::" + k]).ravel()[0])
                                for k in ("variance", "decayTime", "solWeight", "solWeightNorm")])
        m = int(np.asarray(state["turbulence::numModes"]).ravel()[0])
        arr = [np.ascontiguousarray(np.atleast_1d(state["turbulence::" + k]), dtype=np.float64)
               for k in ("modes", "amplitudes", "phases")]
        if [a.size for a in arr] != [3 * m, m, 6 * m]:
            raise ValueError("turbulence state: array sizes do not match numModes")
        rng = state.get("rngEngineState")
        if rng is not None and not isinstance(rng, (bytes, str)):
            rng = np.atleast_1d(rng).astype(np.uint8).tobytes()
        if isinstance(rng, str):
            rng = rng.encode()
        if rng is not None:
            rng = rng.split(b"\0")[0]
        return sc, m, arr, rng

    def _own(self, what):
        if not self.owned:
            raise SxError(f"Turbulence.{what}: this is a Sim's state, a host copy of what the device holds; "
                          "change it with Sim.set_turbulence_state")

    def set_state(self, state):
        self._own("set_state")
        sc, m, arr, rng = self._state_args(state)
        rc = self.L.sx_turb_set_state(self.h, sc, m, *[a.ctypes.data for a in arr], rng)
        if rc != SX_OK:
            raise SxError(f"sx_turb_set_state: code {rc}")

    def max_index(self):
        return int(self.L.sx_turb_max_index(self.h))

    def update_noise(self, dt):
        self._own("update_noise")
        self.L.sx_turb_update_noise(self.h, float(dt))

    def compute_phases(self):
        m = self.num_modes
        re, im = np.empty(3 * m), np.empty(3 * m)
        self.L.sx_turb_compute_phases(self.h, re.ctypes.data, im.ctypes.data)
        return re, im


def stir(ctx, groups, fields, turb):
    ctx.check(ctx.L.sx_stir(ctx.h, C.byref(groups), C.byref(fields), turb.h), "sx_stir")


class Context:
    def __init__(self, device=0, exact=False):
        self.L = lib()
        self.h = C.c_void_p()
        rc = self.L.sx_create(C.byref(self.h), device)
        self.check(rc, "sx_create")
        self.L.sx_set_exact(self.h, 1 if exact else 0)
        self.allocs = []

    def check(self, rc, what=""):
        if rc != SX_OK:
            msg = self.L.sx_last_error(self.h) if self.h else b"?"
            raise SxError(f"{what}: code {rc}: {msg.decode() if msg else ''}")

    def set_exact(self, exact):
        self.L.sx_set_exact(self.h, 1 if exact else 0)

    def alloc(self, n, dtype):
        nbytes = int(n) * np.dtype(dtype).itemsize
        p = self.L.sx_device_alloc(self.h, nbytes)
        if not p:
            raise SxError("device alloc failed")
        self.allocs.append(p)
        return DeviceArray(self, p, int(n), dtype)

    def upload(self, arr):
        arr = np.ascontiguousarray(arr)
        d = self.alloc(arr.size, arr.dtype)
        self.check(self.L.sx_memcpy(self.h, d.ptr, arr.ctypes.data, arr.nbytes, 1), "upload")
        return d

    def free(self, arr):
        if arr.ptr in self.allocs:
            self.allocs.remove(arr.ptr)
            self.L.sx_device_free(self.h, arr.ptr)

    def free_all(self):
        for p in self.allocs:
            self.L.sx_device_free(self.h, p)
        self.allocs = []

    def close(self):
        self.free_all()
        if self.h:
            self.L.sx_destroy(self.h)
            self.h = None

    def sync(self):
        self.check(self.L.sx_synchronize(self.h), "sync")


class DeviceArray:
    def __init__(self, ctx, ptr, n, dtype):
        self.ctx, self.ptr, self.n, self.dtype = ctx, ptr, n, np.dtype(dtype)

    def get(self):
        out = np.empty(self.n, self.dtype)
        self.ctx.check(self.ctx.L.sx_memcpy(self.ctx.h, out.ctypes.data, self.ptr, out.nbytes, 2), "download")
        return out

    def set(self, arr):
        arr = np.ascontiguousarray(arr, dtype=self.dtype)
        assert arr.size == self.n
        self.ctx.check(self.ctx.L.sx_memcpy(self.ctx.h, self.ptr, arr.ctypes.data, arr.nbytes, 1), "upload")


class DeviceState:

    def __init__(self, ctx, host, grad_v=False, std=False):
        self.ctx = ctx
        n = len(host["x"])
        self.n = n
        self.dev = {}
        self.fields = SxFields()
        self.fields.n = n
        grad = ("dV11", "dV12", "dV13", "dV22", "dV23", "dV33")
        for name, _ in FIELD_ORDER:
            if name in ("tdpdTrho", "u", "mue", "mui", "cv", "markRamp", "rung") or \
                    (name in grad and not grad_v) or (name in ("rho", "p") and not std):
                continue
            dt = DTYPES[name]
            if name in host:
                d = ctx.upload(np.asarray(host[name], dtype=dt))
            else:
                d = ctx.alloc(n, dt)
                ctx.L.sx_memset(ctx.h, d.ptr, 0, n * np.dtype(dt).itemsize)
            self.dev[name] = d
            setattr(self.fields, name, d.ptr)

    def get(self, name):
        return self.dev[name].get()

    def set(self, name, arr):
        self.dev[name].set(arr)


class Comm:

    def __init__(self, backend="rccl"):
        import torch
# ... 344 lines not shown
```

Baseline: 1.088 billion.

## Pack neighbor-list local indices into 12-bit fields when union size fits

Cluster-local neighbor indices are stored as 12-bit fields, eight per three 32-bit words, instead of 16-bit halves whenever the cluster's union count is at most 4095. The list writers in neighbor search and skin, and the readers in the hydro, cluster and skin density loops, all switch to the packed layout, with a new software-pipelined unpack loop. The aim is to cut the memory traffic of neighbor-list reads and writes by a quarter. The cost is extra shift and mask work per neighbor, a more complex strided layout, and a fallback path for large unions. It also adds a readfirstlane hint on the wave index.

```diff
diff --git a/include/sphexa_hip.h b/include/sphexa_hip.h
--- a/include/sphexa_hip.h
+++ b/include/sphexa_hip.h
@@ -116,6 +116,10 @@
 int    sx_set_exact(sx_ctx* ctx, int exact);
 double sx_kernel_constant(void);
 int    sx_kernel_poly(const float* v, size_t n, float* w, float* dw);
+int      sx_set_pack12_max(sx_ctx* ctx, uint32_t maxUnion);
+uint32_t sx_pack12_row_words(uint32_t ngmax);
+int      sx_pack12_pack(const uint32_t* pos, uint32_t cnt, uint32_t* words);
+int      sx_pack12_unpack(const uint32_t* words, uint32_t n, uint32_t* pos);
 int    sx_copy_tables(sx_ctx* ctx, float* wh_host, float* whd_host);
 int    sx_synchronize(sx_ctx* ctx);
 
diff --git a/sph-exa_amd/csrc/sx_capi.cpp b/sph-exa_amd/csrc/sx_capi.cpp
--- a/sph-exa_amd/csrc/sx_capi.cpp
+++ b/sph-exa_amd/csrc/sx_capi.cpp
@@ -106,6 +106,7 @@
     hipStream_t own{nullptr};
     hipStream_t stream{nullptr};
     bool        exact{false};
+    int         packMaxSet{-1};
     Arena       arena;
     float2*     wh{nullptr};
     float2*     whd{nullptr};
@@ -127,6 +128,7 @@
     uint32_t powTabNg0{0};
 
     const HydroLaunch& hydro() const { return exact ? hydro_exact() : hydro_fast(); }
+    uint32_t packMax() const { return packMaxSet >= 0 ? (uint32_t)packMaxSet : (exact ? 0u : p12::kPack12Max); }
 };
 
 static const float* ensurePowTab(sx_ctx* c, uint32_t ng0)
@@ -167,6 +169,31 @@
     const float2* sx_ctx_table_internal(sx_ctx* c, int which) { return which ? c->whd : c->wh; }
     const float*  sx_ctx_powtab_internal(sx_ctx* c, uint32_t ng0) { return ensurePowTab(c, ng0); }
     void          sx_ctx_set_error_internal(sx_ctx* c, const char* msg) { fail(c, SX_ERR_ARG, msg); }
+    uint32_t      sx_ctx_pack12_max_internal(sx_ctx* c) { return c->packMax(); }
+
+    int sx_set_pack12_max(sx_ctx* c, uint32_t maxUnion)
+    {
+        if (maxUnion > p12::kPack12Max && maxUnion != 0xffffffffu)
+            return fail(c, SX_ERR_ARG, "sx_set_pack12_max: at most 4095 (or 0xffffffff: the default)");
+        c->packMaxSet = maxUnion == 0xffffffffu ? -1 : (int)maxUnion;
+        return SX_OK;
+    }
+
+    uint32_t sx_pack12_row_words(uint32_t ngmax) { return p12::rowWords(ngmax); }
+
+    int sx_pack12_pack(const uint32_t* pos, uint32_t cnt, uint32_t* words)
+    {
+        for (uint32_t g = 0; g < p12::groups(cnt); ++g)
+            p12::packGroup(pos + p12::kGroup * g, std::min(p12::kGroup, cnt - p12::kGroup * g), words + p12::kWords * g);
+        return SX_OK;
+    }
+
+    int sx_pack12_unpack(const uint32_t* words, uint32_t n, uint32_t* pos)
+    {
+        for (uint32_t k = 0; k < n; ++k)
+            pos[k] = p12::get(words + p12::kWords * (k / p12::kGroup), k % p12::kGroup);
+        return SX_OK;
+    }
 
     int sx_kernel_poly(const float* v, size_t n, float* w, float* dw)
     {
@@ -423,6 +450,7 @@
         a.hitMasks       = c->arena.get<uint64_t>("ns.masks", searchScratchBytes() / sizeof(uint64_t));
         if (!c->nb.reserve(c->arena, first, last, p->ngmax, true) || !a.powTab || !a.clStats || !a.work || !a.hitMasks)
             return fail(c, SX_ERR_NOMEM, "neighbor list allocation failed");
+        c->nb.packMax = c->packMax();
         a.setLists(c->nb);
         SX_HIP(c, hipMemsetAsync(c->stats, 0, kStatsWords * 4, c->stream));
         SX_HIP(c, findNeighbors(a, c->stream));
@@ -540,6 +568,7 @@
     a.uni            = c->nb.uni;
     a.ucount         = c->nb.ucount;
     a.ucap           = c->nb.ucap;
+    a.packMax        = c->nb.packMax;
     a.nc             = f->nc;
     a.rx             = r.rx;
     a.rv             = r.rv;
diff --git a/sph-exa_amd/csrc/sx_device.hpp b/sph-exa_amd/csrc/sx_device.hpp
--- a/sph-exa_amd/csrc/sx_device.hpp
+++ b/sph-exa_amd/csrc/sx_device.hpp
@@ -2,6 +2,8 @@
 
 #include <hip/hip_runtime.h>
 #include <stdint.h>
+
+#include "sx_pack12.hpp"
 
 namespace sx
 {
@@ -13,7 +15,10 @@
 constexpr int kClusterWaves = 4;
 constexpr int kCluster      = kGroupSize * kClusterWaves;
 
-__host__ __device__ constexpr uint32_t nlocWords(uint32_t ngmax) { return (ngmax + 1) / 2; }
+__host__ __device__ constexpr uint32_t nlocWords(uint32_t ngmax)
+{
+    return (ngmax + 1) / 2 > 3 * ((ngmax + 7) / 8) ? (ngmax + 1) / 2 : 3 * ((ngmax + 7) / 8);
+}
 __host__ __device__ constexpr uint32_t unionCap(uint32_t ngmax) { return kCluster * ngmax; }
 
 struct ListsB
diff --git a/sph-exa_amd/csrc/sx_hydro.hip b/sph-exa_amd/csrc/sx_hydro.hip
--- a/sph-exa_amd/csrc/sx_hydro.hip
+++ b/sph-exa_amd/csrc/sx_hydro.hip
@@ -31,8 +31,17 @@
                                       : a.nidx + (size_t)gw * a.ngmax * kWave + lane;                                 \
     const uint32_t* un = a.localLists ? a.uni + (size_t)(gw / kClusterWaves) * a.ucap + (lB ? a.lb.uoff : 0u)        \
                                       : nullptr;                                                                       \
+    const bool p12l = a.localLists && gw < a.numGroups &&                                                             \
+                      (lB ? a.lb.ucount : a.ucount)[gw / kClusterWaves] <= a.packMax;    \
     auto nbj = [&](unsigned k) -> uint32_t {                                                                           \
         if (!a.localLists) return nb[(size_t)k * kWave];                                                               \
+        if (p12l)                                                                                                      \
+        {                                                                                                              \
+            const uint32_t  b = p12::kBits * (k & 7u), t = b >> 5;              \
+            const uint32_t* q = nb + (size_t)(k >> 3) * (p12::kWords * kWave) + (p12::kWords - 1) * lane + t;          \
+            const uint64_t  v = (uint64_t)q[0] | ((uint64_t)q[t < 2 ? 1 : 0] << 32);                                   \
+            return un[(uint32_t)(v >> (b & 31u)) & 0xfffu];                                                            \
+        }                                                                                                              \
         uint32_t w = nb[(size_t)(k >> 1) * kWave];                                                                     \
         return un[(k & 1) ? (w >> 16) : (w & 0xffffu)];                                                                \
     };
diff --git a/sph-exa_amd/csrc/sx_hydro.hpp b/sph-exa_amd/csrc/sx_hydro.hpp
--- a/sph-exa_amd/csrc/sx_hydro.hpp
+++ b/sph-exa_amd/csrc/sx_hydro.hpp
@@ -26,6 +26,7 @@
     const uint32_t* ucount;
     uint32_t        ucap;
     ListsB          lb;
+    uint32_t        packMax;
     const uint32_t* nc;
     const RecX*     rx;
     const RecV*     rv;
diff --git a/sph-exa_amd/csrc/sx_hydro_cluster.hip b/sph-exa_amd/csrc/sx_hydro_cluster.hip
--- a/sph-exa_amd/csrc/sx_hydro_cluster.hip
+++ b/sph-exa_amd/csrc/sx_hydro_cluster.hip
@@ -1,5 +1,6 @@
 #include "sx_hydro.hpp"
 #include "sx_kernel_poly.hpp"
+#include "sx_pack12.hpp"
 #include "sx_traverse.hpp"
 
 namespace sx
@@ -21,7 +22,8 @@
     uint32_t        c, gw, i, iSafe, U;
     bool            valid;
     unsigned        cnt;
-    uint32_t        wBeg, wEnd;
+    uint32_t        gBeg, gEnd;
+    bool            packed;
     int             part;
     int             tid;
     const uint32_t* un;
@@ -67,13 +69,15 @@
         unsigned c1 = a.nc[cu.i] - 1;
         cu.cnt      = c1 < a.ngmax ? c1 : a.ngmax;
     }
-    const uint32_t nw = (cu.cnt + 1) >> 1;
-    cu.wBeg           = nw * cu.part / SPLIT;
-    cu.wEnd           = nw * (cu.part + 1) / SPLIT;
+    const uint32_t ng = p12::groups(cu.cnt);
+    cu.gBeg           = ng * cu.part / SPLIT;
+    cu.gEnd           = ng * (cu.part + 1) / SPLIT;
     const bool lB     = listsB(a.lb, cu.c);
     cu.U              = lB ? a.lb.ucount[cu.c] : a.ucount[cu.c];
+    cu.packed         = cu.U <= a.packMax;
     cu.un             = a.uni + (size_t)cu.c * a.ucap + (lB ? a.lb.uoff : 0u);
-    cu.nl             = (lB ? a.lb.nloc : a.nloc) + (size_t)cu.gw * nlocWords(a.ngmax) * kWave + lane;
+    cu.nl             = (lB ? a.lb.nloc : a.nloc) + (size_t)cu.gw * nlocWords(a.ngmax) * kWave +
+            (cu.packed ? p12::kWords * lane : lane);
     const RecX o      = a.rx[c0];
     cu.ox = o.x, cu.oy = o.y, cu.oz = o.z;
 
@@ -141,7 +145,7 @@
         }
     };
 
-    if (cu.U <= (uint32_t)CH)
+    if (cu.U <= (uint32_t)CH && cu.packed)
     {
         if (!resident)
         {
@@ -149,76 +153,99 @@
             __syncthreads();
             resident = true;
         }
-        const uint32_t wBeg = cu.wBeg, wEnd = cu.wEnd;
-        if (wBeg >= wEnd) return;
-        const uint32_t* nl = cu.nl;
-        if constexpr (LEAN)
-        {
-            const uint32_t wLast = wEnd - 1;
-            auto           ld    = [&](uint32_t w) { return nl[(size_t)min(w, wLast) * kWave]; };
-            constexpr int  D = SX_LEAN_DEPTH;
-            uint32_t       q[D];
-#pragma unroll
-            for (int d = 0; d < D; ++d)
-                q[d] = ld(wBeg + 1 + d);
-            uint32_t       wd = nl[(size_t)wBeg * kWave];
-            auto           ra = load(wd & 0xffffu);
-            for (uint32_t w = wBeg;;)
+        const uint32_t gBeg = cu.gBeg, gEnd = cu.gEnd;
+        if (gBeg >= gEnd) return;
+        const uint32_t gLast = gEnd - 1;
+        struct Grp
+        {
+            uint32_t a, b, c;
+        };
+        auto ldg = [&](uint32_t g) {
+            const uint32_t* p = cu.nl + (size_t)min(g, gLast) * (p12::kWords * kWave);
+            return Grp{p[0], p[1], p[2]};
+        };
+#define SX_P12(E, G) p12::get<E>((G).a, (G).b, (G).c)
+        uint32_t g = gBeg;
+        if constexpr (LEAN || !PF)
+        {
+            const uint32_t* pc  = cu.nl + (size_t)gBeg * (p12::kWords * kWave);
+            uint32_t        rem = min(cu.cnt, p12::kGroup * gEnd) - p12::kGroup * gBeg;
+            uint32_t        w0 = pc[0], w1 = pc[1], w2 = pc[2];
+            auto            r0 = load(p12::get<0>(w0, w1, w2));
+            while (true)
             {
-                const auto rb = load(wd >> 16);
-                compute(ra);
-                const bool odd = 2 * w + 1 < cu.cnt;
-                wd             = q[0];
-#pragma unroll
-                for (int d = 0; d + 1 < D; ++d)
-                    q[d] = q[d + 1];
-                q[D - 1] = ld(w + 1 + D);
-                ra             = load(wd & 0xffffu);
-                if (odd) compute(rb);
-                if (++w >= wEnd) break;
+                pc += rem > p12::kGroup ? p12::kWords * kWave : 0;
+                auto r1 = load(p12::get<1>(w0, w1, w2));
+                compute(r0);
+                const uint32_t p2 = p12::get<2>(w0, w1, w2);
+                w0                = pc[0];
+                r0                = load(p2);
+                if (1 < rem) compute(r1);
+                r1 = load(p12::get<3>(w0, w1, w2));
+                if (2 < rem) compute(r0);
+                r0 = load(p12::get<4>(w0, w1, w2));
+                if (3 < rem) compute(r1);
+                const uint32_t p5 = p12::get<5>(w0, w1, w2);
+                w1                = pc[1];
+                r1                = load(p5);
+                if (4 < rem) compute(r0);
+                r0 = load(p12::get<6>(w0, w1, w2));
+                if (5 < rem) compute(r1);
+                const uint32_t p7 = p12::get<7>(w0, w1, w2);
+                w2                = pc[2];
+                r1                = load(p7);
+                if (6 < rem) compute(r0);
+                r0 = load(p12::get<0>(w0, w1, w2));
+                if (7 < rem) compute(r1);
+                if (rem <= p12::kGroup) break;
+                rem -= p12::kGroup;
             }
             return;
         }
-        const uint32_t  wLast = wEnd - 1;
-        auto            ld    = [&](uint32_t w) {
-            if constexpr (PF) return nl[(size_t)min(w, wLast) * kWave];
-            else return w < wEnd ? nl[(size_t)w * kWave] : 0u;
+        Grp cur = ldg(gBeg), nx = ldg(gBeg + 1);
+        auto         a0 = load(SX_P12(0, cur));
+        auto         b0 = load(SX_P12(1, cur));
+        decltype(a0) a1, b1;
+        while (true)
+        {
+            const uint32_t rem = cu.cnt - p12::kGroup * g;
+            a1 = load(SX_P12(2, cur));
+            b1 = load(SX_P12(3, cur));
+            compute(a0);
+            if (1 < rem) compute(b0);
+            a0 = load(SX_P12(4, cur));
+            b0 = load(SX_P12(5, cur));
+            if (2 < rem) compute(a1);
+            if (3 < rem) compute(b1);
+            a1 = load(SX_P12(6, cur));
+            b1 = load(SX_P12(7, cur));
+            if (4 < rem) compute(a0);
+            if (5 < rem) compute(b0);
+            a0 = load(SX_P12(0, nx));
+            b0 = load(SX_P12(1, nx));
+            if (6 < rem) compute(a1);
+            if (7 < rem) compute(b1);
+            cur = nx;
+            nx  = ldg(g + 2);
+            if (++g >= gEnd) break;
+        }
+#undef SX_P12
+    }
+    else
+    {
+        resident            = false;
+        uint32_t       k    = p12::kGroup * cu.gBeg;
+        const uint32_t kEnd = min(cu.cnt, p12::kGroup * cu.gEnd);
+        auto           pos  = [&](uint32_t k) -> uint32_t {
+            if (cu.packed)
+            {
+                const uint32_t* p    = cu.nl + (size_t)(k >> 3) * (p12::kWords * kWave);
+                const uint32_t  w[3] = {p[0], p[1], p[2]};
+                return p12::get(w, k & 7u);
+            }
+            const uint32_t w = cu.nl[(size_t)(k >> 1) * kWave];
+            return (k & 1) ? (w >> 16) : (w & 0xffffu);
         };
-        uint32_t        q0 = ld(wBeg + 1), q1 = ld(wBeg + 2), q2 = ld(wBeg + 3);
-        const uint32_t  w0 = nl[(size_t)wBeg * kWave];
-        auto            a0 = load(w0 & 0xffffu);
-        auto            b0 = load(w0 >> 16);
-        decltype(a0)    a1, b1;
-        uint32_t        w = wBeg;
-        while (true)
-        {
-            if (PF || w + 1 < wEnd)
-            {
-                a1 = load(q0 & 0xffffu);
-                b1 = load(q0 >> 16);
-                q0 = ld(w + 4);
-            }
-            compute(a0);
-            if (2 * w + 1 < cu.cnt) compute(b0);
-            if (++w >= wEnd) break;
-            if (PF || w + 1 < wEnd)
-            {
-                a0 = load(q1 & 0xffffu);
-                b0 = load(q1 >> 16);
-                q1 = ld(w + 4);
-            }
-            compute(a1);
-            if (2 * w + 1 < cu.cnt) compute(b1);
-            if (++w >= wEnd) break;
-            const uint32_t t = q0;
-            q0 = q2, q2 = q1, q1 = t;
-        }
-    }
-    else
-    {
-        resident         = false;
-        uint32_t       k    = 2 * cu.wBeg;
-        const uint32_t kEnd = min(cu.cnt, 2 * cu.wEnd);
         for (uint32_t b0 = 0; b0 < cu.U; b0 += CH)
         {
             const uint32_t b1 = min(cu.U, b0 + (uint32_t)CH);
@@ -227,8 +254,7 @@
             __syncthreads();
             while (k < kEnd)
             {
-                const uint32_t w = cu.nl[(size_t)(k >> 1) * kWave];
-                const uint32_t p = (k & 1) ? (w >> 16) : (w & 0xffffu);
+                const uint32_t p = pos(k);
                 if (p >= b1) break;
                 compute(load(p - b0));
                 ++k;
@@ -749,7 +775,7 @@
     __shared__ float  s_red[kClusterWaves * SPLIT];
     using Pre                  = MePre<CH, SPLIT, AVC>;
     constexpr int  NT          = Pre::NT, S = Pre::S, SP = Pre::SP;
-    const int      wave        = threadIdx.x >> 6, lane = threadIdx.x & 63;
+    const int      wave        = __builtin_amdgcn_readfirstlane(threadIdx.x >> 6), lane = threadIdx.x & 63;
     const int      sub         = wave & (kClusterWaves - 1);
     const int      part        = wave / kClusterWaves;
     const int      tid         = sub * kWave + lane;
@@ -825,12 +851,14 @@
             const unsigned c1 = cur.nc - 1;
             cu.cnt            = c1 < a.ngmax ? c1 : a.ngmax;
         }
-        const uint32_t nw = (cu.cnt + 1) >> 1;
-        cu.wBeg           = nw * cu.part / SPLIT;
-        cu.wEnd           = nw * (cu.part + 1) / SPLIT;
+        const uint32_t ng = p12::groups(cu.cnt);
+        cu.gBeg           = ng * cu.part / SPLIT;
+        cu.gEnd           = ng * (cu.part + 1) / SPLIT;
         cu.U              = cur.U;
+        cu.packed         = cu.U <= a.packMax;
         cu.un             = a.uni + (size_t)cu.c * a.ucap + (cur.lB ? a.lb.uoff : 0u);
-        cu.nl             = (cur.lB ? a.lb.nloc : a.nloc) + (size_t)cu.gw * nlocWords(a.ngmax) * kWave + lane;
+        cu.nl             = (cur.lB ? a.lb.nloc : a.nloc) + (size_t)cu.gw * nlocWords(a.ngmax) * kWave +
+                (cu.packed ? p12::kWords * lane : lane);
         const RecX o      = cur.o;
         cu.ox = o.x, cu.oy = o.y, cu.oz = o.z;
         const RecX  ri  = cu.valid ? cur.ri : o;
diff --git a/sph-exa_amd/csrc/sx_neighbors.hip b/sph-exa_amd/csrc/sx_neighbors.hip
--- a/sph-exa_amd/csrc/sx_neighbors.hip
+++ b/sph-exa_amd/csrc/sx_neighbors.hip
@@ -888,6 +888,38 @@
         __syncthreads();
         expandFinal();
         if (stored & 1u) ll[(size_t)(stored >> 1) * kWave] = pend;
+        if (ucnt <= a.packMax)
+        {
+            constexpr uint32_t G     = 4;
+            uint32_t* const    row   = ll - lane;
+            const uint32_t     ngr   = p12::groups(stored);
+            const uint32_t     lastW = stored ? (stored - 1u) >> 1 : 0u;
+            __builtin_amdgcn_s_waitcnt(0);
+            for (uint32_t g = 0; g < ngr; g += G)
+            {
+                uint32_t v[4 * G];
+#pragma unroll
+                for (uint32_t t = 0; t < 4 * G; ++t)
+                    v[t] = ll[(size_t)min(4 * g + t, lastW) * kWave];
+                __builtin_amdgcn_fence(__ATOMIC_SEQ_CST, "wavefront");
+                __builtin_amdgcn_s_waitcnt(0);
+                __builtin_amdgcn_wave_barrier();
+#pragma unroll
+                for (uint32_t q = 0; q < G; ++q)
+                {
+                    if (g + q < ngr)
+                    {
+                        uint32_t p[8], w[3];
+#pragma unroll
+                        for (uint32_t t = 0; t < 4; ++t)
+                            p[2 * t] = v[4 * q + t] & 0xffffu, p[2 * t + 1] = v[4 * q + t] >> 16;
+                        p12::packGroup(p, min(8u, stored - 8 * (g + q)), w);
+                        uint32_t* const o = row + ((size_t)(g + q) * kWave + lane) * p12::kWords;
+                        storeList(o, w[0]), storeList(o + 1, w[1]), storeList(o + 2, w[2]);
+                    }
+                }
+            }
+        }
     }
 
     if (valid && !abandoned)
@@ -940,9 +972,21 @@
         {
             if (a.localLists)
             {
-                const bool lB = listsB(a.lb, c);
-                uint32_t   w  = (lB ? a.lb.nloc : a.nloc)[((size_t)g * W + k / 2) * kWave + lane];
-                j = a.uni[(size_t)c * a.ucap + (lB ? a.lb.uoff : 0u) + ((k & 1) ? (w >> 16) : (w & 0xffffu))];
+                const bool      lB  = listsB(a.lb, c);
+                const uint32_t* row = (lB ? a.lb.nloc : a.nloc) + (size_t)g * W * kWave;
+                uint32_t        p;
+                if ((lB ? a.lb.ucount[c] : a.ucount[c]) <= a.packMax)
+                {
+                    const uint32_t* q    = row + ((size_t)(k >> 3) * kWave + lane) * p12::kWords;
+                    const uint32_t  w[3] = {q[0], q[1], q[2]};
+                    p                    = p12::get(w, k & 7u);
+                }
+                else
+                {
+                    const uint32_t w = row[(size_t)(k / 2) * kWave + lane];
+                    p                = (k & 1) ? (w >> 16) : (w & 0xffffu);
+                }
+                j = a.uni[(size_t)c * a.ucap + (lB ? a.lb.uoff : 0u) + p];
             }
             else { j = a.nidx[((size_t)g * a.ngmax + k) * kWave + lane]; }
         }
diff --git a/sph-exa_amd/csrc/sx_pack12.hpp b/sph-exa_amd/csrc/sx_pack12.hpp
--- /dev/null
+++ b/sph-exa_amd/csrc/sx_pack12.hpp
@@ -0,0 +1,51 @@
+#pragma once
+
+#include <hip/hip_runtime.h>
+#include <stdint.h>
+
+namespace sx
+{
+namespace p12
+{
+
+constexpr uint32_t kBits      = 12;
+constexpr uint32_t kGroup     = 8;
+constexpr uint32_t kWords     = 3;
+constexpr uint32_t kPack12Max = 4095;
+
+__host__ __device__ constexpr uint32_t groups(uint32_t cnt) { return (cnt + kGroup - 1) / kGroup; }
+__host__ __device__ constexpr uint32_t rowWords(uint32_t ngmax) { return kWords * groups(ngmax); }
+
+template<int E>
+__host__ __device__ inline uint32_t get(uint32_t w0, uint32_t w1, uint32_t w2)
+{
+    static_assert(E >= 0 && E < 8);
+    if constexpr (E == 0) return w0 & 0xfffu;
+    else if constexpr (E == 1) return (w0 >> 12) & 0xfffu;
+    else if constexpr (E == 2) return ((w0 >> 24) | (w1 << 8)) & 0xfffu;
+    else if constexpr (E == 3) return (w1 >> 4) & 0xfffu;
+    else if constexpr (E == 4) return (w1 >> 16) & 0xfffu;
+    else if constexpr (E == 5) return ((w1 >> 28) | (w2 << 4)) & 0xfffu;
+    else if constexpr (E == 6) return (w2 >> 8) & 0xfffu;
+    else return w2 >> 20;
+}
+
+__host__ __device__ inline uint32_t get(const uint32_t* w, uint32_t e)
+{
+    const uint32_t b = kBits * e, t = b >> 5, s = b & 31u;
+    const uint64_t v = (uint64_t)w[t] | ((uint64_t)w[t < 2 ? t + 1 : 2] << 32);
+    return (uint32_t)(v >> s) & 0xfffu;
+}
+
+__host__ __device__ inline void packGroup(const uint32_t* p, uint32_t n, uint32_t* w)
+{
+    uint32_t q[kGroup];
+    for (uint32_t e = 0; e < kGroup; ++e)
+        q[e] = p[e < n ? e : n - 1] & 0xfffu;
+    w[0] = q[0] | (q[1] << 12) | (q[2] << 24);
+    w[1] = (q[2] >> 8) | (q[3] << 4) | (q[4] << 16) | (q[5] << 28);
+    w[2] = (q[5] >> 4) | (q[6] << 8) | (q[7] << 20);
+}
+
+}
+}
diff --git a/sph-exa_amd/csrc/sx_sim.cpp b/sph-exa_amd/csrc/sx_sim.cpp
--- a/sph-exa_amd/csrc/sx_sim.cpp
+++ b/sph-exa_amd/csrc/sx_sim.cpp
@@ -26,6 +26,7 @@
 
 extern "C" void*          sx_ctx_stream_internal(sx_ctx* c);
 extern "C" int            sx_ctx_exact_internal(sx_ctx* c);
+extern "C" uint32_t       sx_ctx_pack12_max_internal(sx_ctx* c);
 extern "C" const float2*  sx_ctx_table_internal(sx_ctx* c, int which);
 extern "C" const float*   sx_ctx_powtab_internal(sx_ctx* c, uint32_t ng0);
 extern "C" sx::Transport* sx_comm_transport_internal(sx_comm* c);
@@ -625,6 +626,7 @@
     a.uni            = s->nb.uni;
     a.ucount         = s->nb.ucount;
     a.ucap           = s->nb.ucap;
+    a.packMax        = s->nb.packMax;
     a.nc             = s->nc;
     a.rx             = s->rx;
     a.rv             = s->rv;
@@ -1612,6 +1614,7 @@
     fa.x = na.x, fa.y = na.y, fa.z = na.z, fa.h = na.h, fa.m = na.m, fa.nc = na.nc, fa.rxOut = na.rxOut;
     const uint32_t uoff = na.ucap / 2;
     fa.nloc = na.nloc, fa.uni = na.uni, fa.ucount = na.ucount, fa.ucap = na.ucap, fa.uoff = uoff, fa.ucountS = ucS;
+    fa.packMax = na.packMax;
     fa.sloc = sloc, fa.scnt = scnt, fa.hb = hb, fa.rel = rel, fa.acc = acc, fa.cells = cells, fa.grid = g;
     fa.dispX = dx, fa.dispY = dy, fa.dispZ = dz;
     fa.xmOut = xmOut, fa.rtXm = rtXm, fa.K = s->p.K;
@@ -1630,6 +1633,7 @@
     b.skin1    = 1.0f + K.built;
     b.iterateH = 0;
     b.nloc     = sloc;
+    b.packMax  = 0;
     b.ngmax    = K.ngmaxS;
     b.nc       = scnt;
     b.rxOut    = nullptr;
@@ -1947,6 +1951,7 @@
         s->dbox   = toDevBox(box);
         s->bucket = bucketSize;
         s->cap    = capacity;
+        s->nb.packMax = sx_ctx_pack12_max_internal(ctx);
         allocFields(s, capacity);
         if (s->p.propagator == 2) allocBdt(s);
         if (s->mem.failed())
diff --git a/sph-exa_amd/csrc/sx_skin.hip b/sph-exa_amd/csrc/sx_skin.hip
--- a/sph-exa_amd/csrc/sx_skin.hip
+++ b/sph-exa_amd/csrc/sx_skin.hip
@@ -329,7 +329,47 @@
         (void)stage(setUnion(lcur), ue);
         count  = valid ? a.nc[i] - 1u : 0u;
         stored = min(count, a.ngmax);
-        if (a.xmOut && valid)
+        if (a.xmOut && valid && ue <= a.packMax)
+        {
+            const float     hInv = 1.0f / hi, hInv2 = hInv * hInv;
+            const uint32_t  ngr = p12::groups(stored), lastG = ngr ? ngr - 1 : 0u;
+            const uint32_t* lp  = ll + (p12::kWords - 1) * lane;
+            constexpr int   PW  = 2 * p12::kWords;
+            auto            lw  = [&](uint32_t g0, int u) {
+                return lp[(size_t)min(g0 + u / p12::kWords, lastG) * (p12::kWords * kWave) + u % p12::kWords];
+            };
+            uint32_t nx[PW];
+#pragma unroll
+            for (int u = 0; u < PW; ++u)
+                nx[u] = lw(0, u);
+            for (uint32_t g0 = 0; g0 < ngr; g0 += 2)
+            {
+                uint32_t cw[PW];
+#pragma unroll
+                for (int u = 0; u < PW; ++u)
+                {
+                    cw[u] = nx[u];
+                    nx[u] = lw(g0 + 2, u);
+                }
+#pragma unroll
+                for (int h2 = 0; h2 < 2; ++h2)
+                {
+                    const uint32_t w0 = cw[3 * h2], w1 = cw[3 * h2 + 1], w2 = cw[3 * h2 + 2];
+                    const uint32_t pos[8] = {p12::get<0>(w0, w1, w2), p12::get<1>(w0, w1, w2), p12::get<2>(w0, w1, w2),
+                                             p12::get<3>(w0, w1, w2), p12::get<4>(w0, w1, w2), p12::get<5>(w0, w1, w2),
+                                             p12::get<6>(w0, w1, w2), p12::get<7>(w0, w1, w2)};
+#pragma unroll
+                    for (uint32_t e = 0; e < 8; ++e)
+                    {
+                        const float4 q  = s_rec[min(pos[e], (uint32_t)kSkinCap - 1u)];
+                        const float  dx = q.x - xr, dy = q.y - yr, dz = q.z - zr;
+                        const float  r2 = fmaf(dx, dx, fmaf(dy, dy, dz * dz));
+                        rho0 += keepOrZero(kernelWt(r2 * hInv2) * q.w, 8 * (g0 + h2) + e < stored);
+                    }
+                }
+            }
+        }
+        else if (a.xmOut && valid)
         {
             const float    hInv = 1.0f / hi, hInv2 = hInv * hInv;
             const uint32_t nw = (stored + 1) >> 1, last = nw ? nw - 1 : 0u;
@@ -571,7 +611,37 @@
         }
         __syncthreads();
     }
-    if (!kept)
+    if (!kept && ue <= a.packMax)
+    {
+        uint32_t* lw = setLists(ltgt) + (p12::kWords - 1) * lane;
+        uint32_t  acc = 0, nb = 0, t = 0, n = 0, lastR = 0, bits = 0;
+        auto      push = [&](uint32_t r, bool keep) {
+            acc |= keep ? r << nb : 0u;
+            nb += keep ? p12::kBits : 0u;
+            n += keep ? 1u : 0u;
+            if (nb >= 32u)
+            {
+                lw[t] = acc;
+                nb -= 32u;
+                acc = r >> (p12::kBits - nb);
+                if (++t == p12::kWords) t = 0, lw += p12::kWords * kWave;
+            }
+        };
+        walk([&](uint32_t b) { bits = s_bm[b][threadIdx.x]; },
+             [&](uint32_t p, int e, bool) {
+                 const bool keep = ((bits >> e) & 1u) != 0;
+                 lastR           = keep ? s_rank[p] : lastR;
+                 push(lastR, keep);
+             },
+             [](uint32_t) {});
+        while (n & (p12::kGroup - 1u))
+            push(lastR, true);
+        if (uint32_t* const hm = setMask(ltgt))
+            for (uint32_t k = 0; 2 * k < nbl; ++k)
+                hm[(size_t)k * kWave] = maskWord(k);
+        if (threadIdx.x == 0) *setCount(ltgt) = ue;
+    }
+    else if (!kept)
     {
         uint32_t* const lw = setLists(ltgt);
         unsigned st = 0;
diff --git a/sph-exa_amd/csrc/sx_skin.hpp b/sph-exa_amd/csrc/sx_skin.hpp
--- a/sph-exa_amd/csrc/sx_skin.hpp
+++ b/sph-exa_amd/csrc/sx_skin.hpp
@@ -24,6 +24,7 @@
     uint32_t*    nc;
     RecX*        rxOut;
     uint32_t*       nloc;
+    uint32_t        packMax;
     uint32_t*       uni;
     uint32_t*       ucount;
     uint32_t        ucap;
diff --git a/sph-exa_amd/csrc/sx_tree.hpp b/sph-exa_amd/csrc/sx_tree.hpp
--- a/sph-exa_amd/csrc/sx_tree.hpp
+++ b/sph-exa_amd/csrc/sx_tree.hpp
@@ -117,6 +117,7 @@
     uint32_t* nloc{nullptr};
     uint32_t* uni{nullptr};
     uint32_t* ucount{nullptr};
+    uint32_t  packMax{4095};
 
     size_t groups() const { return (size_t(last - first) + kGroupSize - 1) / kGroupSize; }
     size_t clusters() const { return (size_t(last - first) + kCluster - 1) / kCluster; }
@@ -182,6 +183,7 @@
     uint32_t*       uni;
     uint32_t*       ucount;
     uint32_t        ucap;
+    uint32_t        packMax;
     const int32_t*  childOffsets;
     const int32_t*  internalToLeaf;
     const uint32_t* layout;
@@ -218,6 +220,7 @@
         uni        = L.uni;
         ucount     = L.ucount;
         ucap       = L.ucap;
+        packMax    = L.packMax;
     }
 };
 
diff --git a/sph-exa_amd/python/sphexa_amd/__init__.py b/sph-exa_amd/python/sphexa_amd/__init__.py
--- a/sph-exa_amd/python/sphexa_amd/__init__.py
+++ b/sph-exa_amd/python/sphexa_amd/__init__.py
@@ -129,6 +129,10 @@
         "sx_kernel_constant": (C.c_double, []),
         "sx_copy_tables": (C.c_int, [vp, vp, vp]),
         "sx_kernel_poly": (C.c_int, [vp, C.c_size_t, vp, vp]),
+        "sx_set_pack12_max": (C.c_int, [vp, u32]),
+        "sx_pack12_row_words": (u32, [u32]),
+        "sx_pack12_pack": (C.c_int, [vp, u32, vp]),
+        "sx_pack12_unpack": (C.c_int, [vp, u32, vp]),
         "sx_synchronize": (C.c_int, [vp]),
         "sx_device_alloc": (vp, [vp, sz]),
         "sx_device_free": (C.c_int, [vp, vp]),
@@ -448,6 +452,10 @@
     def set_exact(self, exact):
         self.L.sx_set_exact(self.h, 1 if exact else 0)
 
+    def set_pack12_max(self, max_union=None):
+        v = 0xffffffff if max_union is None else int(max_union)
+        self.check(self.L.sx_set_pack12_max(self.h, v), "sx_set_pack12_max")
+
     def alloc(self, n, dtype):
         nbytes = int(n) * np.dtype(dtype).itemsize
         p = self.L.sx_device_alloc(self.h, nbytes)
```

New measurement: 1.141 billion, median of 6. 1.05x the previous value.
